# yjb6/SaRO-GS

Measured on AMD Instinct MI355X. Metric: rendered views/s (fwd+bwd) at 1080p vs #Gaussians, higher is better.
Workload: dtype f32; 1 GPU; BASELINE configs[4] stress-1080p: synth(P=3000000, seed 0) SH3, 1920x1080, one view per GPU, fwd+bwd; protocol=SURVEY 8d: 1 / median of per-call device-synchronised wall-clock fwd+bwd, pose_table=off for value (every pose a first visit); on for value_warm, gaussians=3000000, width=1920, height=1080, sh_degree=3, exp_mode=0, poses_per_rank=8, late_gaussians_cold=2255988, word_fork=0

## Files before the change

### saro-gs_amd/csrc/gsrast_binning.h

```cpp
#pragma once
#include "gsrast_common.h"

namespace gsrast {
#define GSRAST_OCC_ATTR(n) __attribute__((amdgpu_waves_per_eu(n, n)))
#ifdef GSRAST_RSCAT_WAVES
#define GSRAST_RSCAT_OCC GSRAST_OCC_ATTR(GSRAST_RSCAT_WAVES)
#else
#define GSRAST_RSCAT_OCC
#endif
#ifdef GSRAST_BSCAT_WAVES
#define GSRAST_BSCAT_OCC GSRAST_OCC_ATTR(GSRAST_BSCAT_WAVES)
#else
#define GSRAST_BSCAT_OCC
#endif
#ifdef GSRAST_BSORT_WAVES
#define GSRAST_BSORT_OCC GSRAST_OCC_ATTR(GSRAST_BSORT_WAVES)
#else
#define GSRAST_BSORT_OCC
#endif
#ifdef GSRAST_EMIT_WAVES
#define GSRAST_EMIT_OCC GSRAST_OCC_ATTR(GSRAST_EMIT_WAVES)
#else
#define GSRAST_EMIT_OCC
#endif
// ... 472 lines not shown
        for (uint32_t c0 = threadIdx.x; c0 < cgx * cgy; c0 += 256 * 4) {
            uint32_t v[4][4];
#pragma unroll
            for (int u = 0; u < 4; u++) {
                const uint32_t c = c0 + u * 256, cx = c % cgx, cy = c / cgx;
#pragma unroll
                for (int k = 0; k < 4; k++) {
                    const uint32_t x = cx * 2u + (k & 1), y = cy * 2u + (k >> 1);
                    v[u][k] = (c < cgx * cgy && x < gx_tiles && y < gy_tiles) ? zcut_used[y * gx_tiles + x] : 0u;
                }
            }
#pragma unroll
            for (int u = 0; u < 4; u++) {
                const uint32_t c = c0 + u * 256;
                const uint32_t m = max(max(v[u][0], v[u][1]), max(v[u][2], v[u][3]));
                if (c < cgx * cgy) s_zc[c] = (uint16_t)(m >= 0xFFFF0000u ? 0xFFFFu : (m + 0xFFFFu) >> 16);
            }
        }
    }
    SCAT_T(1);
    __syncthreads();
    SCAT_T(2);
    const float scale = (float)nb / (float)s_C[ZH_BINS];
    if (blockIdx.x == 0 && threadIdx.x == 0) *zbins_out = s_fl[0] == 0xFFFFu ? 0xFFFFFFFFu : (s_fl[0] | (s_fl[1] << 16));

    uint32_t dg[BK_ITEMS_T], lr[BK_ITEMS_T];
#pragma unroll
    for (int r = 0; r < BK_ITEMS_T; r++) {
        dg[r] = 0u; lr[r] = 0u;
        if (key[r] != 0xFFFFFFFFu) {
            uint32_t bin, pos; int wlog;
            zh_locate(key[r], zh_klo, zh_shift, bin, pos, wlog);
            const float fscale = __uint_as_float((uint32_t)(127 - wlog) << 23);
            const uint32_t fr = pos;
            const uint32_t c0 = s_C[bin], c1 = s_C[bin + 1u];
            const float u = __builtin_fmaf((float)(c1 - c0), fminf((float)fr * fscale, 0.99999994f), (float)c0);
            const uint32_t d = (uint32_t)(u * scale);
            dg[r] = d < nb ? d : nb - 1u;
            const uint32_t cb = COARSE ? dg[r] >> BK_CSHIFT : dg[r];
            const uint32_t sh = (cb & 1u) * 16u;
            lr[r] = (atomicAdd(&cnt[cb >> 1], 1u << sh) >> sh) & 0xFFFFu;
        }
    }
    uint2 rc[BK_ITEMS_T]; uint32_t tl[BK_ITEMS_T];
#pragma unroll
    for (int r = 0; r < BK_ITEMS_T; r++) {
        const uint32_t i = base + r * 256 + threadIdx.x;
        rc[r] = make_uint2(0u, 0u); tl[r] = 0u;
        if (i < n) { rc[r] = rect[i]; tl[r] = tiles[i]; }
    }
    SCAT_T(3);
    __syncthreads();
    SCAT_T(4);
    const uint32_t nres = COARSE ? nb >> BK_CSHIFT : nb;
    uint32_t* gc = gcount + (size_t)xcd * (COARSE ? (uint32_t)BK_NBC_MAX : nb);
    for (uint32_t k0 = threadIdx.x; k0 < nres; k0 += 256 * 16) {
        uint32_t g[16];
#pragma unroll
        for (int u = 0; u < 16; u++) {
            const uint32_t k = k0 + u * 256;
            const uint32_t c = k < nres ? (cnt[k >> 1] >> ((k & 1u) * 16u)) & 0xFFFFu : 0u;
            g[u] = 0xFFFFFFFFu;
            if (c) g[u] = atomicAdd(&gc[k], c);
        }
#pragma unroll
        for (int u = 0; u < 16; u++) {
            const uint32_t mine = g[u] < 0xFFFFu ? g[u] : 0xFFFFu;
            const uint32_t other = (uint32_t)__shfl_xor((int)mine, 1, 64);
            const uint32_t k = k0 + u * 256;
            if (!(threadIdx.x & 1u) && k < nres) cnt[k >> 1] = mine | (other << 16);
        }
    }
    SCAT_T(5);
    __syncthreads();
    SCAT_T(6);
    uint32_t nlate = 0;
#pragma unroll
    for (int r = 0; r < BK_ITEMS_T; r++) {
        bool skipped = true;
        if (key[r] != 0xFFFFFFFFu) {
            uint32_t wword = (rc[r].y & 0xFFFFu) - (rc[r].x & 0xFFFFu);
            if (zcut_used) {
                const uint32_t x0 = rc[r].x & 0xFFFFu, y0 = rc[r].x >> 16, x1 = rc[r].y & 0xFFFFu, y1 = rc[r].y >> 16;
                const uint32_t kq = key[r] >> 16;
                bool late = wword != 0u && (x1 - x0) * (y1 - y0) <= 64u;
                if (late) {
                    const uint32_t cx0 = x0 >> cshift, cx1 = (x1 - 1u) >> cshift, cy0 = y0 >> cshift, cy1 = (y1 - 1u) >> cshift;
                    uint32_t m = 0;
                    if (cx1 - cx0 <= 1u && cy1 - cy0 <= 1u)
                        m = max(max((uint32_t)s_zc[cy0 * cgx + cx0], (uint32_t)s_zc[cy0 * cgx + cx1]), max((uint32_t)s_zc[cy1 * cgx + cx0], (uint32_t)s_zc[cy1 * cgx + cx1]));
                    else
                        for (uint32_t cy = cy0; cy <= cy1; cy++)
                            for (uint32_t cx = cx0; cx <= cx1; cx++) m = max(m, (uint32_t)s_zc[cy * cgx + cx]);
                    late = kq > m;
                }
                if (late) { wword |= LATE_BIT; nlate++; }
            }
            const uint32_t cb = COARSE ? dg[r] >> BK_CSHIFT : dg[r];
            const uint32_t pos = ((cnt[cb >> 1] >> ((cb & 1u) * 16u)) & 0xFFFFu) + lr[r];
            if (COARSE) {
#ifdef GSRAST_SCAT_BATCH_STORES
                rc[r].x = wword | ((dg[r] & ((1u << BK_CSHIFT) - 1u)) << 16);
                lr[r] = pos;
#else
                if (pos < ccap)
                    slab[((size_t)cb * BK_XCD + xcd) * ccap + pos] = make_uint4(key[r], base + r * 256 + threadIdx.x, wword | ((dg[r] & ((1u << BK_CSHIFT) - 1u)) << 16), tl[r]);
#endif
            } else if (pos < (uint32_t)BK_CAPX)
                slab[((size_t)dg[r] * BK_XCD + xcd) * BK_CAPX + pos] = make_uint4(key[r], base + r * 256 + threadIdx.x, wword, tl[r]);
            skipped = (wword & LATE_BIT) != 0u;
        }
        if (color_skip) {
            const unsigned long long m = __ballot(skipped);
            const uint32_t first = base + r * 256 + (threadIdx.x & ~63u);
            if (lane == 0 && first < n) color_skip[first >> 6] = m;
        }
    }
#ifdef GSRAST_SCAT_BATCH_STORES
    if (COARSE) {
#pragma unroll
        for (int r = 0; r < BK_ITEMS_T; r++)
            if (key[r] != 0xFFFFFFFFu && lr[r] < ccap)
                slab[((size_t)(dg[r] >> BK_CSHIFT) * BK_XCD + xcd) * ccap + lr[r]] = make_uint4(key[r], base + r * 256 + threadIdx.x, rc[r].x, tl[r]);
    }
#endif
    if (zcut_used) {
#pragma unroll
        for (int d = 32; d >= 1; d >>= 1) nlate += __shfl_xor(nlate, d, 64);
        if (lane == 0 && nlate) atomicAdd(&s_late, nlate);
        __syncthreads();
        if (threadIdx.x == 0 && s_late) atomicAdd(n_late_out, s_late);
    }
    SCAT_T(7);
#ifdef GSRAST_SCATTER_TIMING
    if (threadIdx.x == 0) atomicMax(&g_scat[13], (unsigned long long)wall_clock64());
#endif
    {
        const uint32_t per = (nb + gridDim.x) / gridDim.x;
        const uint32_t b = blockIdx.x * per + threadIdx.x;
        if (threadIdx.x < per && b <= nb) {
            const float u = (float)b * ((float)s_C[ZH_BINS] / (float)nb);
            uint32_t i = 0;
#pragma unroll
            for (uint32_t st = ZH_BINS / 2; st; st >>= 1) if ((float)s_C[i + st] <= u) i += st;
            const long long k0 = zh_bin_start(i, zh_klo, zh_shift), k1 = zh_bin_start(i + 1u, zh_klo, zh_shift);
            const float c0 = (float)s_C[i], c1 = (float)s_C[i + 1u];
            const float f = fminf(fmaxf((u - c0) / (c1 - c0), 0.0f), 1.0f);
            const long long k = k0 + (long long)(f * (float)(k1 - k0));
            bkey_out[b] = k < 0 ? 0u : (k < (long long)ZH_KEY_TOP ? (uint32_t)k : ZH_KEY_TOP);
        }
    }
}

__global__ void __launch_bounds__(256)
depth_bucket_refine_kernel(const uint4* __restrict__ cslab , const uint32_t* __restrict__ gccount , uint32_t nb,
                           uint32_t* __restrict__ gcount , uint4* __restrict__ slab , uint32_t ccap)
{
    __shared__ uint32_t cnt[1 << BK_CSHIFT];
    const uint32_t x = blockIdx.x & (BK_XCD - 1), c = blockIdx.x >> 3;
    if (threadIdx.x < (1u << BK_CSHIFT)) cnt[threadIdx.x] = 0u;
    const uint32_t n_true = gccount[(size_t)x * BK_NBC_MAX + c];
    const uint32_t n = n_true < ccap ? n_true : ccap;
    const uint4* src = cslab + ((size_t)c * BK_XCD + x) * ccap;
    constexpr int RI = 8;
    __syncthreads();
    for (uint32_t e0 = 0; e0 < n; e0 += RI * 256) {
        uint4 el[RI];
#pragma unroll
        for (int r = 0; r < RI; r++) { const uint32_t e = e0 + r * 256 + threadIdx.x; if (e < n) el[r] = src[e]; }
#pragma unroll
        for (int r = 0; r < RI; r++) {
            const uint32_t e = e0 + r * 256 + threadIdx.x;
            if (e < n) {
                const uint32_t fb = (el[r].z >> 16) & ((1u << BK_CSHIFT) - 1u);
                const uint32_t pos = atomicAdd(&cnt[fb], 1u);
                if (pos < (uint32_t)BK_CAPX)
                    slab[((size_t)((c << BK_CSHIFT) + fb) * BK_XCD + x) * BK_CAPX + pos] = make_uint4(el[r].x, el[r].y, el[r].z & ~BK_FINE_MASK, el[r].w);
            }
        }
    }
    __syncthreads();
    if (threadIdx.x < (1u << BK_CSHIFT))
        gcount[(size_t)x * nb + (c << BK_CSHIFT) + threadIdx.x] = (n_true > ccap && threadIdx.x == 0u) ? 0xFFFFu : cnt[threadIdx.x];
}

__device__ __forceinline__ void wave_sync() { __builtin_amdgcn_fence(__ATOMIC_ACQ_REL, "wavefront"); __builtin_amdgcn_wave_barrier(); }
constexpr int BK_SUB = 256;
constexpr int BK_WAVES = 2;

__device__ __forceinline__ uint4 bucket_element(const uint4* __restrict__ slab, uint32_t b, const uint32_t (&start)[BK_XCD + 1], uint32_t e)
{
    uint32_t x = 0, s0 = 0;
#pragma unroll
    for (int q = 1; q < BK_XCD; q++) { const bool ge = e >= start[q]; x += ge ? 1u : 0u; s0 = ge ? start[q] : s0; }
    return slab[((size_t)b * BK_XCD + x) * BK_CAPX + (e - s0)];
}
__global__ void __launch_bounds__(64 * BK_WAVES) GSRAST_BSORT_OCC
depth_bucket_sort_kernel(const uint4* __restrict__ slab, const uint32_t* __restrict__ gcount, uint32_t nb,
                         const uint32_t* __restrict__ bkey ,
                         uint32_t* __restrict__ border ,
                         uint32_t* __restrict__ bwincl ,
                         uint4* __restrict__ binfo ,
                         uint32_t* __restrict__ bwsum ,
                         uint4* __restrict__ binfo_all = nullptr,
                         const uint32_t* __restrict__ pred = nullptr ,
                         const unsigned long long* __restrict__ keep_bits = nullptr,
                         uint32_t* __restrict__ zero_words = nullptr, uint32_t n_zero_words = 0,
                         uint4* __restrict__ zero_quads = nullptr, uint32_t n_zero_quads = 0)
{
    __shared__ unsigned long long s_grp[BK_WAVES][BK_CAP];
    __shared__ uint16_t s_aux[BK_WAVES][BK_CAP];
    __shared__ uint16_t s_wid[BK_WAVES][BK_CAP];
    __shared__ uint32_t s_cnt[BK_WAVES][BK_SUB + 1];
    if (pred && *pred == 0u) return;
    if (zero_words) for (uint32_t k = blockIdx.x * blockDim.x + threadIdx.x; k < n_zero_words; k += gridDim.x * blockDim.x) zero_words[k] = 0u;
    if (zero_quads) for (uint32_t k = blockIdx.x * blockDim.x + threadIdx.x; k < n_zero_quads; k += gridDim.x * blockDim.x) zero_quads[k] = make_uint4(0u, 0u, 0u, 0u);
    const unsigned lane = lane_id(), wave = threadIdx.x >> 6;
    const uint32_t b = blockIdx.x * BK_WAVES + wave;
    if (b >= nb) return;
    const bool early_only = binfo_all != nullptr;
    unsigned long long* grp = s_grp[wave];
    uint16_t* aux = s_aux[wave];
    uint16_t* wid = s_wid[wave];
    uint32_t* cnt = s_cnt[wave];
    const uint32_t sub_lo = bkey[b], sub_hi = bkey[b + 1u];
    const float sub_scale = (float)BK_SUB / (float)(sub_hi > sub_lo ? sub_hi - sub_lo : 1u);
    auto sub_of = [&](uint32_t key) -> uint32_t {
        if (key <= sub_lo) return 0u;
        const uint32_t d = (uint32_t)((float)(key - sub_lo) * sub_scale);
        return d < (uint32_t)BK_SUB ? d : (uint32_t)BK_SUB - 1u;
    };
    uint32_t c = lane < (unsigned)BK_XCD ? gcount[(size_t)lane * nb + b] : 0u;
    const uint32_t over = __ballot(c > (uint32_t)BK_CAPX) != 0ull ? 1u : 0u;
    c = c < (uint32_t)BK_CAPX ? c : (uint32_t)BK_CAPX;
    uint32_t inc = c;
#pragma unroll
    for (int d = 1; d < BK_XCD; d <<= 1) { const uint32_t t = __shfl_up(inc, d, 64); if (lane >= (unsigned)d) inc += t; }
    uint32_t start[BK_XCD + 1];
    start[0] = 0u;
#pragma unroll
    for (int x = 0; x < BK_XCD; x++) start[x + 1] = __builtin_amdgcn_readlane(inc, x);
    const uint32_t n_all = start[BK_XCD];
    for (uint32_t k = lane; k <= (uint32_t)BK_SUB; k += 64) cnt[k] = 0u;
    wave_sync();
    uint32_t tsum = 0, wall = 0;
    for (uint32_t e0 = lane; e0 < n_all; e0 += 64 * 4) {
        uint4 kv[4];
#pragma unroll
        for (int u = 0; u < 4; u++) { const uint32_t e = e0 + u * 64; kv[u] = e < n_all ? bucket_element(slab, b, start, e) : make_uint4(0u, 0u, 0u, 0u); }
#pragma unroll
        for (int u = 0; u < 4; u++) {
            const uint32_t e = e0 + u * 64;
            if (e < n_all) {
                const bool kept = !(early_only && (kv[u].z & LATE_BIT)) && (!keep_bits || ((keep_bits[kv[u].y >> 6] >> (kv[u].y & 63u)) & 1ull));
                if (!keep_bits || kept) tsum += kv[u].w;
                wall += kv[u].z & ~LATE_BIT;
                if (kept) aux[e] = atomicAdd(&cnt[sub_of(kv[u].x)], 1u);
            }
        }
    }
    wave_sync();
    {
        uint32_t v[BK_SUB / 64], sum = 0;
#pragma unroll
        for (int q = 0; q < BK_SUB / 64; q++) { v[q] = cnt[lane * (BK_SUB / 64) + q]; sum += v[q]; }
        uint32_t run = wave_incl_scan(sum) - sum;
#pragma unroll
        for (int q = 0; q < BK_SUB / 64; q++) { cnt[lane * (BK_SUB / 64) + q] = run; run += v[q]; }
        if (lane == 63) cnt[BK_SUB] = run;
    }
    wave_sync();
    const uint32_t n = cnt[BK_SUB];
    for (uint32_t e0 = lane; e0 < n_all; e0 += 64 * 4) {
        uint4 kv[4];
#pragma unroll
        for (int u = 0; u < 4; u++) { const uint32_t e = e0 + u * 64; kv[u] = e < n_all ? bucket_element(slab, b, start, e) : make_uint4(0u, 0u, 0u, 0u); }
#pragma unroll
        for (int u = 0; u < 4; u++) {
            const uint32_t e = e0 + u * 64;
            if (e < n_all && !(early_only && (kv[u].z & LATE_BIT)) && (!keep_bits || ((keep_bits[kv[u].y >> 6] >> (kv[u].y & 63u)) & 1ull))) {
                const uint32_t slot = cnt[sub_of(kv[u].x)] + aux[e];
                grp[slot] = ((unsigned long long)kv[u].x << 32) | kv[u].y;
                wid[slot] = (uint16_t)(kv[u].z & ~LATE_BIT);
            }
        }
    }
    wave_sync();
    for (uint32_t e = lane; e < n; e += 64) {
        const unsigned long long me = grp[e];
        const uint32_t d2 = sub_of((uint32_t)(me >> 32));
        const uint32_t s0 = cnt[d2], s1 = cnt[d2 + 1];
        uint32_t r = 0;
        for (uint32_t q = s0; q < s1; q++) r += grp[q] < me ? 1u : 0u;
        border[(size_t)b * BK_CAP + s0 + r] = (uint32_t)me;
        aux[s0 + r] = wid[e];
    }
    wave_sync();
    const uint32_t E = (n + 63) / 64;
    uint32_t wsum = 0;
    for (uint32_t e = 0; e < E; e++) { const uint32_t t = lane * E + e; if (t < n) wsum += aux[t]; }
    uint32_t run = wave_incl_scan(wsum) - wsum;
    const uint32_t wtot = __shfl(run + wsum, 63, 64);
#pragma unroll
    for (int d = 32; d >= 1; d >>= 1) { tsum += __shfl_xor(tsum, d, 64); wall += __shfl_xor(wall, d, 64); }
    uint32_t* scanbuf = reinterpret_cast<uint32_t*>(grp);
    for (uint32_t e = 0; e < E; e++) { const uint32_t t = lane * E + e; if (t < n) { run += aux[t]; scanbuf[t] = run; } }
    wave_sync();
    for (uint32_t t = lane; t < n; t += 64) bwincl[(size_t)b * BK_CAP + t] = scanbuf[t];
    if (lane == 0) {
        if (early_only) { binfo[b] = make_uint4(n, wtot, n_all - n, over); binfo_all[b] = make_uint4(n_all, wall, tsum, over); }
        else binfo[b] = make_uint4(n, wtot, tsum, over);
        bwsum[b] = wtot;
    }
}

__device__ __forceinline__ void depth_bucket_totals(const uint4* __restrict__ binfo, uint32_t nb, uint32_t* __restrict__ scalars,
                                                    uint32_t* host_out = nullptr, uint32_t host_seq = 0,
                                                    const uint4* __restrict__ binfo_e = nullptr )
{
    __shared__ unsigned long long s_t[256];
    __shared__ uint32_t s_q[256], s_qe[256];
    uint32_t over = 0, q = 0, qe = 0;
    unsigned long long tsum = 0;
    for (uint32_t k0 = threadIdx.x; k0 < nb; k0 += 256 * 8) {
        uint4 v[8];
#pragma unroll
        for (int u = 0; u < 8; u++) { const uint32_t k = k0 + u * 256; v[u] = k < nb ? binfo[k] : make_uint4(0u, 0u, 0u, 0u); }
#pragma unroll
        for (int u = 0; u < 8; u++) { q += v[u].y; tsum += v[u].z; over |= v[u].w; }
        if (binfo_e) {
#pragma unroll
            for (int u = 0; u < 8; u++) { const uint32_t k = k0 + u * 256; v[u] = k < nb ? binfo_e[k] : make_uint4(0u, 0u, 0u, 0u); }
#pragma unroll
            for (int u = 0; u < 8; u++) qe += v[u].y;
        }
    }
    s_t[threadIdx.x] = tsum; s_q[threadIdx.x] = q; s_qe[threadIdx.x] = qe;
    over = __syncthreads_or((int)over) ? 1u : 0u;
    for (int st = 128; st > 0; st >>= 1) { if ((int)threadIdx.x < st) { s_t[threadIdx.x] += s_t[threadIdx.x + st]; s_q[threadIdx.x] += s_q[threadIdx.x + st]; s_qe[threadIdx.x] += s_qe[threadIdx.x + st]; } __syncthreads(); }
    if (threadIdx.x == 0) {
        scalars[SC_R_LO] = (uint32_t)s_t[0]; scalars[SC_Q] = s_q[0]; scalars[SC_R_HI] = (uint32_t)(s_t[0] >> 32); scalars[SC_BUCKET_OVER] = over;
        const uint32_t q_early = binfo_e ? s_qe[0] : s_q[0], n_late = binfo_e ? scalars[SC_N_LATE] : 0u;
        scalars[SC_Q_EARLY] = q_early;
        scalars[SC_EARLY_COUNTS + SC_R_LO] = (uint32_t)s_t[0]; scalars[SC_EARLY_COUNTS + SC_Q] = q_early; scalars[SC_EARLY_COUNTS + SC_LISTED] = 0u; scalars[SC_EARLY_COUNTS + SC_R_HI] = (uint32_t)(s_t[0] >> 32);
        if (host_out) {
            unsigned long long* h64 = reinterpret_cast<unsigned long long*>(host_out);
            uint32_t vals[SC_BUCKET_OVER + 1];
            vals[SC_R_LO] = (uint32_t)s_t[0]; vals[SC_Q] = s_q[0]; vals[SC_BUCKET_OVER] = over; vals[SC_R_HI] = (uint32_t)(s_t[0] >> 32);
            vals[SC_Q_EARLY] = q_early; vals[SC_N_LATE] = n_late; vals[SC_ZBINS] = scalars[SC_ZBINS];
#pragma unroll
            for (int k = 0; k < RB_WORDS; k++)
                __hip_atomic_store(h64 + k, ((unsigned long long)host_seq << 32) | vals[kReadbackWord[k]], __ATOMIC_RELAXED, __HIP_MEMORY_SCOPE_SYSTEM);
        }
    }
}
__global__ void __launch_bounds__(256)
depth_bucket_scan_kernel(const uint4* __restrict__ binfo, uint32_t nb, uint32_t* __restrict__ scalars )
{
    depth_bucket_totals(binfo, nb, scalars);
}

__global__ void __launch_bounds__(256)
cut_candidates_kernel(uint32_t P, const uint32_t* __restrict__ tiles, const uint2* __restrict__ rect, const unsigned char* __restrict__ need2,
                      uint32_t ntiles, uint32_t gx, unsigned long long* __restrict__ skip, unsigned long long* __restrict__ cand,
                      unsigned long long* __restrict__ skip2, const uint32_t* __restrict__ pred)
{
    __shared__ uint32_t s_need[(BUCKET_MAX_TILES + 32) / 32];
    if (pred && *pred == 0u) return;
    const uint32_t nw = (ntiles + 31u) / 32u;
    for (uint32_t w = threadIdx.x; w < nw; w += 256) {
        uint32_t m = 0;
        for (uint32_t k = 0; k < 32u; k++) { const uint32_t t = w * 32u + k; if (t < ntiles && need2[t]) m |= 1u << k; }
        s_need[w] = m;
    }
    __syncthreads();
    for (uint32_t i0 = blockIdx.x * 256u; i0 < ((P + 63u) & ~63u); i0 += gridDim.x * 256u) {
        const uint32_t i = i0 + threadIdx.x;
        bool c = false;
        if (i < P && tiles[i] != 0u) {
            const uint2 rc = rect[i];
            const uint32_t x0 = rc.x & 0xFFFFu, y0 = rc.x >> 16, x1 = rc.y & 0xFFFFu, y1 = rc.y >> 16;
            if ((x1 - x0) * (y1 - y0) > 1024u) c = true;
            else
                for (uint32_t y = y0; y < y1 && !c; y++)
                    for (uint32_t x = x0; x < x1; x++) { const uint32_t t = y * gx + x; if ((s_need[t >> 5] >> (t & 31u)) & 1u) { c = true; break; } }
        }
        const unsigned long long m = __ballot(c);
        if ((threadIdx.x & 63u) == 0u && i < ((P + 63u) & ~63u)) {
            const unsigned long long old = skip[i >> 6];
            cand[i >> 6] = m;
            skip2[i >> 6] = ~(old & m);
            skip[i >> 6] = old & ~m;
        }
    }
}

template <typename KeyT>
__global__ void __launch_bounds__(256)
emit_instances_kernel(int P, const uint32_t* __restrict__ order, const uint32_t* __restrict__ offsets,
                      const uint32_t* __restrict__ tiles, const uint2* __restrict__ rect, int gx,
                      KeyT* __restrict__ tile_keys, uint32_t* __restrict__ inst_vals)
{
    __shared__ uint32_t s_e[4][64], s_g[4][64], s_xy[4][64], s_w[4][64];
    const int j = blockIdx.x * blockDim.x + threadIdx.x;
    const unsigned lane = lane_id(), wave = threadIdx.x >> 6;
    uint32_t g = 0, cnt = 0, incl, xy = 0, w = 1;
    if (j < P) {
        g = order[j];
        cnt = tiles[g];
        incl = offsets[j];
        if (cnt) {
            const uint2 rc = rect[g];
            xy = rc.x;
            w = (rc.y & 0xFFFFu) - (rc.x & 0xFFFFu);
        }
    } else {
        incl = P > 0 ? offsets[P - 1] : 0u;
    }
    const uint32_t e = incl - cnt;
    const uint32_t wstart = __shfl(e, 0, 64);
    const uint32_t wend = __shfl(incl, 63, 64);
    s_e[wave][lane] = e - wstart; s_g[wave][lane] = g; s_xy[wave][lane] = xy; s_w[wave][lane] = w;
    __syncthreads();
    const uint32_t C = wend - wstart;
    for (uint32_t o = lane; o < C; o += 64) {
        uint32_t sidx = 0;
#pragma unroll
        for (int step = 32; step >= 1; step >>= 1)
            if (s_e[wave][sidx + step] <= o) sidx += step;
        const uint32_t k = o - s_e[wave][sidx];
        const uint32_t ww = s_w[wave][sidx], pxy = s_xy[wave][sidx];
        uint32_t yy = (uint32_t)((float)k * __builtin_amdgcn_rcpf((float)ww));
        if (yy * ww > k) yy--;
        if ((yy + 1) * ww <= k) yy++;
        const uint32_t xx = k - yy * ww;
        tile_keys[wstart + o] = (KeyT)(((pxy >> 16) + yy) * (uint32_t)gx + (pxy & 0xFFFFu) + xx);
        inst_vals[wstart + o] = s_g[wave][sidx];
    }
}

template <typename KeyT>
__global__ void __launch_bounds__(256)
tile_ranges_kernel(uint32_t R, const uint32_t* __restrict__ R_dev ,
                   const KeyT* __restrict__ tile_keys_sorted, uint2* __restrict__ ranges)
{
    const uint32_t i = blockIdx.x * blockDim.x + threadIdx.x;
    if (R_dev) R = *R_dev;
    if (i >= R) return;
    const uint32_t cur = tile_keys_sorted[i];
    if (i == 0) ranges[cur].x = 0;
    else {
        const uint32_t prev = tile_keys_sorted[i - 1];
        if (cur != prev) { ranges[prev].y = i; ranges[cur].x = i; }
    }
    if (i == R - 1) ranges[cur].y = R;
}

__device__ __forceinline__ double sqrt_newton(double x)
{
    const float xf = (float)x;
    if (!(xf > 1e-30f) || !(xf < 1e30f)) return sqrt(x);
    const float s0f = __builtin_sqrtf(xf);
    const double s0 = (double)s0f;
// ... 465 lines not shown
```

### saro-gs_amd/csrc/gsrast_capi.hip

```cpp
#include "gsrast_host.h"
#include "gsrast_common.h"
#include "gsrast_policy.h"
#include "gsrast_preprocess.h"
#include "gsrast_binning.h"
#include "gsrast_blend.h"
#include "gsrast_contrib.h"
#include "gsrast_features.h"
#include "gsrast_distort.h"
#include "gsrast_project.h"
#include "gsrast_exchange.h"

#include <algorithm>
#include <atomic>
#include <chrono>
#include <cstdlib>
#include <thread>
#include <cstdio>
#include <cmath>
#include <cstring>
#include <dlfcn.h>
#ifndef GSRAST_LATE_FILL_WGS
#define GSRAST_LATE_FILL_WGS 256
#endif
#include <mutex>
#include <string>
#include <vector>
#include <unordered_map>

using namespace gsrast;

namespace {

thread_local std::string g_err;
enum OptionKind { OPT_FLAG , OPT_ONE_OF , OPT_CLAMP , OPT_WORD  };
struct OptionRow { const char* name; std::atomic<int>* word; int def; OptionKind kind; int a, b; int gsrast_options::* field ; };
constexpr int OPT_01 = 0b11, OPT_012 = 0b111, OPT_PPL = 0b10111 , OPT_MAX = 0x7FFFFFFF;
constexpr OptionRow kOptions[] = {
    { "exp_mode", &g_opt.exp_mode, 0, OPT_ONE_OF, OPT_012, 0, &gsrast_options::exp_mode },
    { "binning", &g_opt.binning, 0, OPT_ONE_OF, OPT_01, 0, &gsrast_options::binning },
    { "tile_clip", &g_opt.tile_clip, 1, OPT_FLAG, 0, 0, &gsrast_options::tile_clip },
    { "cull", &g_opt.cull, 1, OPT_FLAG, 0, 0, &gsrast_options::cull },
    { "lpt", &g_opt.lpt, 1, OPT_FLAG, 0, 0, &gsrast_options::lpt },
    { "speculative", &g_opt.speculative, 1, OPT_FLAG, 0, 0, &gsrast_options::speculative },
    { "fwd_pixels_per_lane", &g_opt.fwd_pixels_per_lane, 0, OPT_ONE_OF, OPT_PPL, 0, &gsrast_options::fwd_pixels_per_lane },
    { "bwd_pixels_per_lane", &g_opt.bwd_pixels_per_lane, 0, OPT_ONE_OF, OPT_PPL, 0, &gsrast_options::bwd_pixels_per_lane },
    { "sh_grad_factors", &g_opt.sh_grad_factors, 0, OPT_FLAG, 0, 0, &gsrast_options::sh_grad_factors },
    { "side_stream", &g_opt.side_stream, 1, OPT_FLAG, 0, 0, &gsrast_options::side_stream },
    { "depth_sort", &g_opt.depth_sort, 0, OPT_ONE_OF, OPT_01, 0, &gsrast_options::depth_sort },
    { "forward_only", &g_opt.forward_only, 0, OPT_FLAG, 0, 0, &gsrast_options::forward_only },
    { "no_order_hint", &g_opt.no_order_hint, 0, OPT_FLAG, 0, 0, &gsrast_options::no_order_hint },
    { "dense_backward", &g_opt.dense_backward, 0, OPT_FLAG, 0, 0, &gsrast_options::dense_backward },
    { "no_list_cut", &g_opt.no_list_cut, 0, OPT_FLAG, 0, 0, &gsrast_options::no_list_cut },
    { "profile", &g_opt.profile, 0, OPT_WORD, 0, 0, nullptr },
    { "debug_sync", &g_opt.debug_sync, 0, OPT_FLAG, 0, 0, nullptr },
    { "debug_state", &g_opt.debug_state, 0, OPT_FLAG, 0, 0, nullptr },
    { "ablate", &g_opt.ablate, 0, OPT_WORD, 0, 0, nullptr },
    { "mutate", &g_opt.mutate, 0, OPT_WORD, 0, 0, nullptr },
    { "list_cut_always", &g_opt.list_cut_always, 0, OPT_FLAG, 0, 0, nullptr },
    { "chain_gate", &g_opt.chain_gate, 1, OPT_FLAG, 0, 0, nullptr },
    { "touch_bits", &g_opt.touch_bits, 1, OPT_FLAG, 0, 0, nullptr },
    { "sparse_grec", &g_opt.sparse_grec, 1, OPT_FLAG, 0, 0, nullptr },
    { "late_fill_min_p", &g_opt.late_fill_min_p, 750000, OPT_CLAMP, 0, OPT_MAX, nullptr },
    { "tau_sample", &g_opt.tau_sample, 1, OPT_CLAMP, 0, 6, nullptr },
    { "tau_cut", &g_opt.tau_cut, 1, OPT_FLAG, 0, 0, nullptr },
    { "two_level", &g_opt.two_level, 1, OPT_FLAG, 0, 0, nullptr },
    { "two_level_min_p", &g_opt.two_level_min_p, 2500000, OPT_CLAMP, 0, OPT_MAX, nullptr },
    { "sort_hint", &g_opt.sort_hint, 1, OPT_FLAG, 0, 0, nullptr },
    { "bwd_transposed", &g_opt.bwd_transposed, 1, OPT_FLAG, 0, 0, nullptr },
    { "hexplane_scatter", &g_opt.hexplane_scatter, 0, OPT_ONE_OF, OPT_01, 0, nullptr },
};
const OptionRow* option_row(const char* name)
{
    for (const OptionRow& r : kOptions) if (!strcmp(name, r.name)) return &r;
    return nullptr;
}
bool option_take(const OptionRow& r, int value, int* stored)
{
    *stored = r.kind == OPT_FLAG ? (value ? 1 : 0) : r.kind == OPT_CLAMP ? std::min(std::max(value, r.a), r.b) : value;
    return r.kind != OPT_ONE_OF || (value >= 0 && value < 31 && ((r.a >> value) & 1) != 0);
}
PlanSwitches snapshot_switches()
{
    const OptionWords& g = g_opt;
    return PlanSwitches{ g.list_cut_always.load() != 0, g.tau_cut.load() != 0, g.touch_bits.load() != 0, g.sparse_grec.load() != 0, g.two_level.load() != 0, g.chain_gate.load() != 0,
                         g.sort_hint.load() != 0, g.debug_state.load() != 0, g.two_level_min_p.load(), g.tau_sample.load(), g.bwd_transposed.load() != 0, g.late_fill_min_p.load(),
                         g.ablate.load(), g.mutate.load() };
}

const char* const kKernelNames[K_COUNT] = { "preprocess_fwd", "sort_depth", "scan_tiles", "emit_instances",
                                            "sort_tile", "tile_ranges", "blend_fwd", "blend_bwd",
                                            "preprocess_bwd", "mark_visible", "loss_fwd", "loss_bwd", "preprocess_color", "sh_dir_derivs",
                                            "cut_redo" ,
                                            "late_rows_zero" ,
                                            "grec_zero_touched" ,
                                            "densify_classify", "densify_scan", "densify_apply", "densify_stats_update" ,
                                            "contrib_blend", "contrib_finish" ,
                                            "features_fwd", "features_bwd" ,
                                            "distort_fwd", "distort_bwd" ,
                                            "adam_step_visible" ,
                                            "mcmc_plan" , "mcmc_sample" ,
                                            "mcmc_apply" , "mcmc_noise" ,
                                            "mlp_fwd" , "mlp_bwd"  };
thread_local int t_prof_off = 0;
struct Pending { int id; hipEvent_t a, b; };
std::mutex g_prof_mu;
std::vector<Pending> g_pending;
double g_total_ms[K_COUNT];
long long g_launches[K_COUNT];

struct Roctx {
    int (*push)(const char*) = nullptr; int (*pop)() = nullptr;
    Roctx()
    {
        if (!getenv("GSRAST_ROCTX")) return;
        void* h = dlopen("librocprofiler-sdk-roctx.so", RTLD_NOW | RTLD_GLOBAL);
        if (!h) h = dlopen("libroctx64.so", RTLD_NOW | RTLD_GLOBAL);
        if (!h) return;
        push = reinterpret_cast<int (*)(const char*)>(dlsym(h, "roctxRangePushA"));
        pop = reinterpret_cast<int (*)()>(dlsym(h, "roctxRangePop"));
        if (!push || !pop) { push = nullptr; pop = nullptr; }
    }
};
const Roctx& roctx() { static const Roctx r; return r; }
}

namespace gsrast {
OptionWords g_opt;
OptionWords::OptionWords() { for (const OptionRow& r : kOptions) r.word->store(r.def); }
gsrast_options snapshot_defaults()
{
    gsrast_options o{};
    for (const OptionRow& r : kOptions) if (r.field) o.*r.field = r.word->load();
    return o;
}

int fail(int code, const char* what, hipError_t e)
{
    char buf[512];
    if (e != hipSuccess) snprintf(buf, sizeof buf, "%s: %s", what, hipGetErrorString(e));
    else snprintf(buf, sizeof buf, "%s", what);
    g_err = buf;
    return code;
}

RoctxRange::RoctxRange(const char* name) : on(roctx().push != nullptr) { if (on) (void)roctx().push(name); }
RoctxRange::~RoctxRange() { if (on) (void)roctx().pop(); }

ProfScope::ProfScope(int id_, hipStream_t s_) : id(id_), s(s_), on((id_ < 32 ? ((g_opt.profile.load() >> id_) & 1) != 0 : g_opt.profile.load() == -1) && (t_prof_off == 0 || id_ == K_CUT_REDO)), range(kKernelNames[id_])
{
    if (on) { (void)hipEventCreate(&a); (void)hipEventCreate(&b); (void)hipEventRecord(a, s); }
}
ProfScope::~ProfScope()
{
    if (on) {
        (void)hipEventRecord(b, s);
        std::lock_guard<std::mutex> lk(g_prof_mu);
        g_pending.push_back({ id, a, b });
    }
}

int post_launch(const char* what, hipStream_t s)
{
    hipError_t e = hipGetLastError();
    if (e != hipSuccess) return fail(GSRAST_E_DEVICE, what, e);
    static const bool env_sync = getenv("GSRAST_DEBUG_SYNC") != nullptr;
    if (g_opt.debug_sync.load() || env_sync) {
        if (env_sync) fprintf(stderr, "[gsrast] %s\n", what);
        e = hipStreamSynchronize(s);
        if (e != hipSuccess) return fail(GSRAST_E_DEVICE, what, e);
    }
    return GSRAST_OK;
}
}

namespace {
int scan_u32(const uint32_t* src, const uint32_t* idx, uint32_t n, uint32_t* dst, bool inclusive,
             uint32_t* tmp, uint32_t* total_out, hipStream_t s, const uint2* runs = nullptr,
             const uint32_t* aux = nullptr, uint32_t* aux_lo = nullptr, uint32_t* aux_hi = nullptr)
{
    if (n == 0) return GSRAST_OK;
    const uint32_t nb = (n + SC_CHUNK - 1) / SC_CHUNK;
    if (nb == 1 && !aux) {
        scan_apply_kernel<<<1, 256, 0, s>>>(src, idx, runs, n, nullptr, dst, inclusive ? 1 : 0, total_out);
        GS_LAUNCHED("scan_apply");
        return GSRAST_OK;
    }
    scan_block_sums_kernel<<<nb, 256, 0, s>>>(src, idx, runs, n, tmp, aux, tmp + nb);
    GS_LAUNCHED("scan_block_sums");
    scan_single_block_kernel<<<1, 256, 0, s>>>(tmp, nb, aux ? tmp + nb : nullptr, aux_lo, aux_hi);
    GS_LAUNCHED("scan_single_block");
    scan_apply_kernel<<<nb, 256, 0, s>>>(src, idx, runs, n, tmp, dst, inclusive ? 1 : 0, total_out);
    GS_LAUNCHED("scan_apply");
    return GSRAST_OK;
}

template <typename KeyT, typename ValT> struct SortAdapt { KeyT* kC; ValT* vC; uint32_t* block_minmax; uint32_t* sig; bool assume_short; };

template <typename KeyT, typename ValT = uint32_t, int ITEMS = RS_ITEMS>
int radix_sort(KeyT* kA, ValT* vA, KeyT* kB, ValT* vB, uint32_t n, int bits,
               uint32_t* hist, uint32_t* scan_tmp, hipStream_t s,
               const uint2* gather_rect = nullptr, uint32_t* gather_tiles = nullptr, uint32_t* gather_width = nullptr,
               const uint32_t* n_dev = nullptr ,
               const SortAdapt<KeyT, ValT>* ad = nullptr, const uint32_t* pred = nullptr )
{
    if (n == 0) return GSRAST_OK;
    const uint32_t nblk = (n + RS_THREADS * ITEMS - 1) / (RS_THREADS * ITEMS);
    const int passes = radix_passes(bits);
    if (ad && passes == 4 && bits == 32 && nblk > RS_SELF_SCAN_BLOCKS) {
        const uint32_t mask = 255u;
        const int as = ad->assume_short ? RA_ASSUME : 0;
        for (int p = 0; p < (ad->assume_short ? 3 : 4); p++) {
            const int shift = 8 * p;
            const KeyT* kin = (p & 1) ? kB : kA; const ValT* vin = (p & 1) ? vB : vA;
            KeyT* kout = (p & 1) ? kA : kB; ValT* vout = (p & 1) ? vA : vB;
            const int hmode = (p == 0 ? RA_MINMAX : p == 2 ? RA_IN_ALT : p == 3 ? RA_SKIP : 0) | as;
            const int smode = (p == 1 ? RA_OUT_ALT : p == 2 ? (RA_IN_ALT | RA_OUT_ALT | RA_LAST_IF_SHORT) : p == 3 ? RA_SKIP : 0) | as;
            radix_hist_kernel<KeyT, ITEMS><<<nblk, RS_THREADS, 0, s>>>(kin, n, n_dev, shift, mask, hist, nblk, ad->kC, p ? ad->sig : nullptr, hmode, ad->block_minmax);
            GS_LAUNCHED("radix_hist");
            radix_rowscan_kernel<<<mask + 1 + (p == 0 ? 1 : 0), 256, 0, s>>>(hist, nblk, scan_tmp, ad->sig, (p == 0 ? RA_MINMAX : p == 3 ? RA_SKIP : 0) | as, ad->block_minmax, mask + 1);
            GS_LAUNCHED("radix_rowscan");
            radix_scatter_kernel<KeyT, ValT, ITEMS><<<nblk, RS_THREADS, 0, s>>>(kin, vin, kout, vout, n, n_dev, shift, mask, hist, scan_tmp, nblk,
                                                                         p >= 2 ? gather_rect : nullptr, gather_tiles, gather_width,
                                                                         ad->kC, ad->vC, p == 1 ? ad->kC : kA, p == 1 ? ad->vC : vA, ad->sig, smode);
            GS_LAUNCHED("radix_scatter");
        }
        return GSRAST_OK;
    }
    int shift = 0;
    for (int p = 0; p < passes; p++) {
        const int w = (bits - shift + (passes - p) - 1) / (passes - p);
        const uint32_t mask = (1u << w) - 1u;
        radix_hist_kernel<KeyT, ITEMS><<<nblk, RS_THREADS, 0, s>>>(kA, n, n_dev, shift, mask, hist, nblk, nullptr, nullptr, 0, nullptr, pred);
        GS_LAUNCHED("radix_hist");
        const bool self_scan = nblk <= RS_SELF_SCAN_BLOCKS;
        if (!self_scan) {
            radix_rowscan_kernel<<<mask + 1, 256, 0, s>>>(hist, nblk, scan_tmp, nullptr, 0, nullptr, 0, pred);
            GS_LAUNCHED("radix_rowscan");
        }
        const bool last = p == passes - 1;
// ... 376 lines not shown
            blend_fwd_kernel<MODE, PPL><<<grid, 256 / PPL, 0, s>>>(a.ranges, a.plist, a.W, a.H, a.gx, a.T, a.r0, a.r1, a.r2, a.bg, a.oc, a.od, a.fT, a.nc, a.tm, a.bcnt, a.blist);
        });
    });
}

void launch_blend_bwd(int exp_mode, const BlendBwdPick& k, uint32_t grid, hipStream_t s, const BlendArgs& a)
{
    const uint32_t* bcnt = a.from_buckets ? a.bcnt : nullptr;
    auto uncull = [&](auto mode, auto lanes, auto abl) {
        constexpr int PPL = decltype(lanes)::value;
        blend_bwd_kernel<decltype(mode)::value, PPL, decltype(abl)::value><<<grid, 256 / PPL, 0, s>>>(a.ranges, a.plist, a.W, a.H, a.gx, a.T, a.r0, a.r1, a.r2, a.bg, a.fT, a.nc, a.tm, a.dpix, a.grec);
    };
    if (k.ablate) return pick_int<1, 2>(k.ablate, [&](auto abl) { uncull(int_c<0>{}, int_c<4>{}, abl); });
    pick_int<0, 1, 2>(exp_mode, [&](auto mode) {
        constexpr int MODE = decltype(mode)::value;
        if (k.transposed) pick_bool(k.aux, [&](auto aux) { pick_bool(k.abs, [&](auto abs_c) {
            constexpr bool AUX = decltype(aux)::value, ABS = decltype(abs_c)::value;
            blend_bwd_cull_t_kernel<MODE, AUX, ABS><<<grid, 256, 0, s>>>(a.ranges, a.plist, a.order, a.W, a.H, a.gx, a.T, a.r0, a.r1, a.r2, a.bg, a.fT, a.nc, a.tm, a.dpix, a.grec,
                                                                         bcnt, a.blist, AUX ? a.dad : nullptr, AUX ? a.dal : nullptr);
        }); });
        else if (k.cull) pick_int<4, 2, 1>(k.ppl, [&](auto lanes) {
            constexpr int PPL = decltype(lanes)::value;
            blend_bwd_cull_kernel<MODE, PPL><<<grid, 256 / PPL, 0, s>>>(a.ranges, a.plist, a.order, a.W, a.H, a.gx, a.T, a.r0, a.r1, a.r2, a.bg, a.fT, a.nc, a.tm, a.dpix, a.grec, bcnt, a.blist);
        });
        else pick_int<4, 2, 1>(k.ppl, [&](auto lanes) { uncull(mode, lanes, int_c<0>{}); });
    });
}

struct ReplayLaunch {
    int W, H, gx; uint32_t T; unsigned grid;
    const uint2* ranges; const uint32_t* point_list;
    const float4 *rec0, *rec1; const float* final_T; const uint32_t *n_contrib, *tile_max;
    size_t grec;
    ReplayLaunch(int P, int width, int height, const char* geom, const char* binning, const char* image)
    {
        const GeomLayout GL = geom_layout((size_t)P);
        const ImgLayout IL = img_layout((size_t)width, (size_t)height);
        W = width; H = height; gx = (width + TILE_X - 1) / TILE_X;
        T = (uint32_t)gx * (uint32_t)((height + TILE_Y - 1) / TILE_Y); grid = ((T + 7) / 8) * 8;
        ranges = at<uint2>(image, IL.ranges); point_list = at<uint32_t>(binning, 0);
        rec0 = at<float4>(geom, GL.rec0); rec1 = at<float4>(geom, GL.rec1); grec = GL.grec;
        final_T = at<float>(image, IL.final_T); n_contrib = at<uint32_t>(image, IL.n_contrib); tile_max = at<uint32_t>(image, IL.tile_max);
    }
    template <class K, class... A> void front_to_back(K kernel, hipStream_t s, A... own) const
    { kernel<<<grid, 256, 0, s>>>(ranges, point_list, W, H, gx, T, rec0, rec1, n_contrib, tile_max, own...); }
    template <class K, class... A> void back_to_front(K kernel, hipStream_t s, A... own) const
    { kernel<<<grid, 256, 0, s>>>(ranges, point_list, W, H, gx, T, rec0, rec1, final_T, n_contrib, tile_max, own...); }
};

}

extern "C" {

int gsrast_abi_version(void) { return GSRAST_ABI_VERSION; }
const char* gsrast_last_error(void) { return g_err.c_str(); }

void gsrast_options_init(gsrast_options* o)
{
    if (!o) return;
    memset(o, 0, sizeof *o);
    for (const OptionRow& r : kOptions) if (r.field) o->*r.field = r.def;
}
gsrast_context* gsrast_context_create(void) { return new (std::nothrow) gsrast_context(); }
void gsrast_context_destroy(gsrast_context* c)
{
    if (!c) return;
    for (DeviceState& d : c->dev) d.release();
    delete c;
}
int gsrast_context_query(const gsrast_context* c, const char* name)
{
    if (!name) return GSRAST_E_ARG;
    if (!c) c = thread_context();
    if (!strcmp(name, "last_instances")) return (int)c->last_R.load();
    if (!strcmp(name, "last_runs")) return (int)c->last_Q.load();
    if (!strcmp(name, "last_prologue_ns")) return (int)c->last_prologue_ns.load();
    if (!strcmp(name, "redo_count")) return c->redo_count.load();
    if (!strcmp(name, "bucket_skip")) return c->zsort.skip.load();
    if (!strcmp(name, "last_late")) return (int)c->last_late.load();
    if (!strcmp(name, "last_early_runs")) return (int)c->last_Qe.load();
    if (!strcmp(name, "completion_passes")) return (int)c->pol.passes_reported.load();
    if (!strcmp(name, "tau_req")) return c->pol.tau_req.load();
    if (!strcmp(name, "tau_force")) return c->pol.tau_force.load();
    if (!strcmp(name, "cut_margin_x4")) return c->pol.margin.load();
    if (!strcmp(name, "gate_inline_calls")) {
        const int device = current_device();
        return device < 0 ? 0 : (int)c->dev[device].gate.inline_calls;
    }
    if (!strcmp(name, "cut_pause")) return c->pol.pause.load();
    if (!strcmp(name, "cut_fallbacks")) {
        const int device = current_device();
        if (device < 0) return 0;
        if (hipDeviceSynchronize() != hipSuccess) return GSRAST_E_DEVICE;
        uint32_t sum = 0;
        for (const auto& h : c->dev[device].hints) {
            uint32_t v = 0;
            if (h.table && hipMemcpy(&v, &h.table->cut_fallbacks, sizeof v, hipMemcpyDeviceToHost) != hipSuccess) return GSRAST_E_DEVICE;
            sum += v;
        }
        return (int)sum;
    }
    return GSRAST_E_ARG;
}

int gsrast_policy_event(gsrast_context* c, const char* what, int a, int b, int c3)
{
    if (!what) return GSRAST_E_ARG;
    if (!c) c = thread_context();
    CutPolicy& pol = c->pol;
    if (!strcmp(what, "begin")) {
        pol.begin_forward((uint32_t)a);
        c->last_R = (uint32_t)a;
        const bool pays = pol.pays((uint32_t)b, c3 != 0);
        if (!pays) pol.sits_out();
        return pays ? 1 : 0;
    }
    if (!strcmp(what, "counts")) { pol.forward_counts((c3 & 1) != 0, (c3 & 2) ? 1u : 0u, (uint32_t)a, (uint32_t)b, c->last_R.load(), false); return pol.pause.load(); }
    if (!strcmp(what, "pass")) return pol.completion_pass((uint32_t)a, (uint32_t)b, c->last_R.load(), false, c3 != 0);
    if (!strcmp(what, "clean")) { pol.clean_cut_forward(); return pol.fb_score.load(); }
    if (!strcmp(what, "size")) return (int)early_launch_runs((uint32_t)a, (uint32_t)b, c3 != 0);
    if (!strcmp(what, "grow")) return (int)grow_capacity((uint32_t)a);
    if (!strcmp(what, "follow")) return (int)follow_hint((uint32_t)a, (uint32_t)b, c3);
    if (!strcmp(what, "depth_sort")) {
        if (a == 0) c->zsort.radix_forward(); else if (a == 1) c->zsort.clean_forward(); else if (a == 2) (void)c->zsort.overflow(b != 0); else return GSRAST_E_ARG;
        return c->zsort.skip.load();
    }
    if (!strcmp(what, "reset")) { c->pol.~CutPolicy(); new (&c->pol) CutPolicy(); c->zsort.~DepthSortPolicy(); new (&c->zsort) DepthSortPolicy(); return 0; }
    if (!strcmp(what, "tau_min")) { pol.tau_min = std::max(1, a); pol.tau_req = std::max(1, a); return a; }
    if (!strcmp(what, "zrange")) {
        const uint32_t k = c->zrange.klo.load(); const int sh = c->zrange.shift.load();
        const bool held = c->zrange.learn((uint32_t)a, k, sh);
        return c->zrange.shift.load() | (held ? 256 : 0);
    }
    if (!strcmp(what, "zget")) return a == 0 ? (int)(c->zrange.klo.load() >> 8) : a == 1 ? c->zrange.shift.load() : (int)(c->zrange.khi.load() >> 8);
    if (!strcmp(what, "get")) {
        switch (a) { case 0: return pol.pause.load(); case 1: return pol.fb_score.load(); case 2: return pol.margin.load(); case 3: return pol.tau_req.load();
                     case 4: return pol.tau_force.load(); case 5: return pol.fb_pause.load();
                     case 6: return c->zsort.skip.load(); case 7: return c->zsort.backoff.load(); case 8: return c->zsort.clean.load(); default: return GSRAST_E_ARG; }
    }
    return GSRAST_E_ARG;
}

int gsrast_debug_forward_plan(gsrast_context* c, const gsrast_options* options, unsigned flags, int P, int W, int H, const int* words)
{
    if (!options || !words) return fail(GSRAST_E_ARG, "debug_forward_plan: NULL argument");
    if (!c) c = thread_context();
    ForwardPlan p = plan_forward(*options, PlanInputs{ flags, P, W, H, words[4] >> 4, (words[4] & 1) != 0, (words[4] & 2) != 0, words[0], (uint32_t)words[1], (uint32_t)words[2], words[3] != 0 }, snapshot_switches());
    if (p.refusal) return fail(GSRAST_E_ARG, p.refusal);
    p.policy_answer(c->pol.pays(p.last_Q, p.list_cut_always), words[5] != 0);
    const bool bits[] = { p.runbin, p.buckets_ok, p.bucket_sort, p.two_level, p.culled, p.ordered, p.want_hints, p.cut_base, p.tau_mode, p.zero_in_blend, p.zero_touched,
                          p.keep_untouched, p.clip, p.want_shd, p.spec_eligible, p.adaptive_sort, p.assume_short, p.cut_pays, p.cut };
    int v = 0;
    for (size_t k = 0; k < sizeof bits / sizeof bits[0]; k++) v |= bits[k] ? 1 << k : 0;
    return v;
}

int gsrast_debug_backward_plan(const gsrast_options* options, unsigned flags, const int* words, int* grids)
{
    if (!options || !words) return fail(GSRAST_E_ARG, "debug_backward_plan: NULL argument");
    const int in = words[5];
    BackwardInputs bi{ flags, words[0], words[1], words[2], words[3], words[4], (in & 1) != 0, (in & 2) != 0, (in & 4) != 0, (in & 8) != 0, (in & 16) != 0 };
    bi.known_flags = backward_known_flags((in & 32) ? sizeof(gsrast_backward_call) : GSRAST_BACKWARD_CALL_MIN);
    bi.pose_out = (in & 64) != 0; bi.pose_scratch = (in & 128) != 0; bi.abs_sink = (in & 256) != 0;
    BackwardPlan p = plan_backward(*options, bi, snapshot_switches());
    if (p.refusal) return fail(GSRAST_E_ARG, p.refusal);
    p.side_answer(p.wants_side() && words[6] != 0);
    if (grids) { grids[0] = p.derivs_grid; grids[1] = p.per_gaussian_grid; }
    const bool bits[] = { p.aux, p.aa, p.do_blend, p.do_geom, p.zero_records, p.derivs, p.derivs_on_side, p.late_fill_wanted, p.late_fill, p.skip_zero_rows, p.join_late,
                          p.blend, p.pick.cull, p.pick.transposed, p.pick.aux, p.from_buckets, p.tile_order, p.sh_factor, p.factors != 0, p.sparse, p.grouped };
    int v = 0;
    for (size_t k = 0; k < sizeof bits / sizeof bits[0]; k++) v |= bits[k] ? 1 << k : 0;
    return v | p.pick.ppl << 21 | p.pick.ablate << 24 | (p.mutate & 3) << 26 | (p.pose ? 1 << 28 : 0);
}

int gsrast_set_option(const char* name, int value)
{
    if (!name) return GSRAST_E_ARG;
    if (!strcmp(name, "word_fork")) return value == 0 ? 0 : GSRAST_E_ARG;
    const bool both = !strcmp(name, "pixels_per_lane");
    const OptionRow* r = option_row(both ? "fwd_pixels_per_lane" : name);
    int stored = 0;
    if (!r || !option_take(*r, value, &stored)) return GSRAST_E_ARG;
    r->word->store(stored);
    if (both) g_opt.bwd_pixels_per_lane = stored;
    return 0;
}
int gsrast_get_option(const char* name)
{
    if (!name) return GSRAST_E_ARG;
    if (!strcmp(name, "word_fork")) return 0;
    for (const char* word : { "last_instances", "last_runs", "redo_count", "bucket_skip" }) if (!strcmp(name, word)) return gsrast_context_query(nullptr, name);
    const OptionRow* r = option_row(!strcmp(name, "pixels_per_lane") ? "fwd_pixels_per_lane" : name);
    return r ? r->word->load() : GSRAST_E_ARG;
}

int gsrast_profile_kernel_count(void) { return K_COUNT; }
const char* gsrast_profile_kernel_name(int id) { return (id >= 0 && id < K_COUNT) ? kKernelNames[id] : ""; }
int gsrast_profile_collect(void)
{
    std::lock_guard<std::mutex> lk(g_prof_mu);
    for (auto& p : g_pending) {
        float ms = 0.f;
        if (hipEventSynchronize(p.b) == hipSuccess && hipEventElapsedTime(&ms, p.a, p.b) == hipSuccess) {
            g_total_ms[p.id] += ms; g_launches[p.id] += 1;
        }
        (void)hipEventDestroy(p.a); (void)hipEventDestroy(p.b);
    }
    g_pending.clear();
    return 0;
}
int gsrast_profile_read(int id, double* total_ms, long long* launches)
{
    if (id < 0 || id >= K_COUNT) return GSRAST_E_ARG;
    std::lock_guard<std::mutex> lk(g_prof_mu);
    if (total_ms) *total_ms = g_total_ms[id];
    if (launches) *launches = g_launches[id];
    return 0;
}
void gsrast_profile_reset(void)
{
    gsrast_profile_collect();
    std::lock_guard<std::mutex> lk(g_prof_mu);
    for (int i = 0; i < K_COUNT; i++) { g_total_ms[i] = 0; g_launches[i] = 0; }
}

size_t gsrast_geometry_bytes(int P) { return geom_layout((size_t)(P > 0 ? P : 0)).total; }
size_t gsrast_binning_bytes(int R, int, int) { return bin_layout((size_t)(R > 0 ? R : 0)).total; }
size_t gsrast_image_bytes(int W, int H) { return img_layout((size_t)(W > 0 ? W : 0), (size_t)(H > 0 ? H : 0)).total; }
void* gsrast_alloc_prealloc(void* ctx, size_t bytes)
{
    gsrast_prealloc* p = static_cast<gsrast_prealloc*>(ctx);
    if (!p) return nullptr;
    p->requested = bytes;
    return bytes <= p->capacity ? p->ptr : nullptr;
}

int gsrast_mark_visible(int P, const float* means3D, const float* viewmatrix, const float* projmatrix,
                        unsigned char* present, void* stream)
{
    (void)projmatrix;
    hipStream_t s = (hipStream_t)stream;
    if (P < 0 || (P > 0 && (!means3D || !viewmatrix || !present))) return fail(GSRAST_E_ARG, "mark_visible: NULL argument");
    if (P == 0) return GSRAST_OK;
    ProfScope ps(K_MARK_VISIBLE, s);
    mark_visible_kernel<<<(P + 255) / 256, 256, 0, s>>>(P, means3D, viewmatrix, present);
    GS_LAUNCHED("mark_visible");
    return GSRAST_OK;
}

static int prefilter_verdict(const uint32_t* word, hipStream_t s)
{
    uint32_t v = 0;
    GS_HIP(hipMemcpyAsync(&v, word, sizeof v, hipMemcpyDeviceToHost, s));
    GS_HIP(hipStreamSynchronize(s));
    return v ? fail(GSRAST_E_ARG, "forward: a Gaussian passed as prefiltered was culled by the near plane (the reference traps: auxiliary.h:156-160)") : GSRAST_OK;
}

static const char* raw_inputs_check(int P, int M, const gsrast_raw_inputs* in)
{
    if (!in) return "raw: NULL inputs";
    if (P == 0) return nullptr;
    if (!in->xyz || !in->rotation || !in->scaling || !in->opacity_logit || !in->features_dc || (M > 1 && !in->features_rest)) return "raw: NULL required input";
    if (M < 1 || M * 3 > PP_SH_MAX || ((M * 3) & 3)) return "raw: M must be 4 or 16 (SH rows of a multiple of 16 bytes, at most 16 coefficients)";
    if (((uintptr_t)in->rotation | (uintptr_t)in->features_dc | (uintptr_t)in->features_rest | (uintptr_t)in->shs_res) & 15) return "raw: rotation / features_dc / features_rest / shs_res must be 16-byte aligned";
    return nullptr;
}

extern "C++" { namespace {
struct BucketSortArgs {
    const uint4* slab; const uint32_t* gcount; uint32_t nb; const uint32_t* bkey; uint32_t *border, *bwincl; uint4* binfo; uint32_t* bwsum;
    uint4* binfo_all = nullptr;
    const uint32_t* pred = nullptr; const unsigned long long* keep_bits = nullptr;
    uint32_t* zero_words = nullptr; uint32_t n_zero_words = 0; uint4* zero_quads = nullptr; uint32_t n_zero_quads = 0;
};
void launch_bucket_sort(hipStream_t s, const BucketSortArgs& a)
{
    depth_bucket_sort_kernel<<<(a.nb + BK_WAVES - 1) / BK_WAVES, 64 * BK_WAVES, 0, s>>>(a.slab, a.gcount, a.nb, a.bkey, a.border, a.bwincl, a.binfo, a.bwsum, a.binfo_all, a.pred, a.keep_bits,
                                                                                   a.zero_words, a.n_zero_words, a.zero_quads, a.n_zero_quads);
}
struct EmitArgs {
    uint32_t grid; int P; const uint32_t *order, *woffsets; const float4* binrec; int W, H, clip; uint32_t capQ; uint16_t* run_keys; uint2* run_vals;
    const float4 *rec0, *rec1; const uint2* rect;
    const uint4* binfo = nullptr; const uint32_t* bwsum = nullptr; uint32_t nbuckets = 0;
    uint32_t* scalars = nullptr; uint32_t* host_out = nullptr; uint32_t host_seq = 0;
    const uint4* binfo_all = nullptr; const uint32_t* pred = nullptr;
    uint32_t* redo_bucket_cnt = nullptr; int n_redo_cnt = 0; HintTable* redo_hints = nullptr; unsigned long long* host_fallback = nullptr; uint32_t host_fb_seq = 0;
    const unsigned char* need2 = nullptr; int gx_tiles = 0; uint32_t* pass2_counts = nullptr;
};
void launch_emit(hipStream_t s, const EmitArgs& a)
{
    emit_column_runs_kernel<<<a.grid, 256, 0, s>>>(a.P, a.order, a.woffsets, a.binrec, a.W, a.H, a.clip, a.capQ, a.run_keys, a.run_vals, a.binfo, a.bwsum, a.nbuckets, a.scalars,
                                               a.host_out, a.host_seq, a.binfo_all, a.pred, a.redo_bucket_cnt, a.n_redo_cnt, a.redo_hints, a.host_fallback, a.host_fb_seq,
                                               a.need2, a.gx_tiles, a.pass2_counts, a.rec0, a.rec1, a.rect);
}
bool trace_on() { static const bool on = getenv("GSRAST_TRACE") != nullptr; return on; }

struct ForwardRun {
    gsrast_context* const ctx; const gsrast_forward_call& c; const gsrast_options o; const std::chrono::steady_clock::time_point t_entry; const hipStream_t stream;
    const int device; DeviceState* const dev;
    ForwardPlan plan;
    const float *means3D, *shs, *opacities, *scales, *rotations;
    const gsrast_raw_inputs* rawin = nullptr; RawArgs raw{};
    float *out_acc_depth = nullptr, *out_alpha = nullptr;
    int P = 0, W = 0, H = 0; uint32_t T = 0, nbk = 0; CamArgs cam;
    GeomLayout GL; ImgLayout IL; char *geom = nullptr, *img = nullptr, *bin = nullptr; uint32_t cap = 0, capQ = 0;
    float4 *rec0, *rec1, *rec2, *binrec, *grec; uint32_t* tiles; uint2* rect; uint32_t *kA, *kB, *vA, *vB, *offsets, *woffsets, *hist, *scan_tmp, *scalars, *hint_sel, *prefilter_word;
    uint4 *bk_slab, *bk_info, *bk_info_e; uint32_t *bk_count, *bk_key, *bk_order, *bk_wincl, *bk_base, *bk_order_e, *bk_wincl_e, *bk_base_e;
    unsigned long long *color_skip, *cand_bits; unsigned char *untouched = nullptr, *tile_flags; uint32_t* bucket_cnt; uint16_t* bucket_list; uint2* ranges;
    uint32_t *zcut_used = nullptr, *tau_hist = nullptr, *zhist_call = nullptr; TauBins tau_bins{};
    HintTable* hints = nullptr;
    uint32_t zh_klo = 0, zh_wave_mask = 0; int zh_shift = 0;
    uint32_t *zhist_ctx = nullptr, *tau_ctx = nullptr;
    struct SideJoinGuard {
        SideStream* side = nullptr; bool launched = false , joined = false;
        ~SideJoinGuard() { if (launched && side && !joined) (void)hipStreamSynchronize(side->stream); }
    } fork;
    bool bucketed = false;
    bool totals_pending = false;
    bool sort_redone = false;
    Readback *rb_pre = nullptr, *rb_flag = nullptr, *rb = nullptr; uint32_t *pre_alias = nullptr, *flag_alias = nullptr; uint32_t pre_seq = 0, flag_seq = 0;
    ChainGate* gate = nullptr; uint32_t gseq = 0, *gdone = nullptr, *gpred = nullptr;
    uint32_t counts[kCountWords] = { 0 }; uint32_t nQ1 = 0;
    std::chrono::steady_clock::time_point t0, t1;

    ForwardRun(gsrast_context* ctx_, const gsrast_options* options, const gsrast_forward_call& c_, std::chrono::steady_clock::time_point t)
        : ctx(ctx_ ? ctx_ : thread_context()), c(c_), o(options ? *options : snapshot_defaults()), t_entry(t), stream((hipStream_t)c_.stream),
          device(current_device()), dev(ctx->device_state(device)), means3D(c_.means3D), shs(c_.shs), opacities(c_.opacities), scales(c_.scales), rotations(c_.rotations) {}

    int check_and_plan(hipStream_t s)
    {
        P = c.P; W = c.width; H = c.height;
        const bool raw_family = c.family == GSRAST_FAMILY_RAW;
        plan = plan_forward(o, PlanInputs{ c.flags, P, W, H, c.D, (raw_family ? c.raw && c.raw->features_dc : c.shs != nullptr), c.colors_precomp != nullptr,
                                           ctx->zsort.skip.load(), ctx->R_hint.load(), ctx->last_Q.load(), ctx->zsort.depth_short.load() != 0 }, snapshot_switches());
        if (plan.refusal) return fail(GSRAST_E_ARG, plan.refusal);
        if (plan.aux) { out_acc_depth = c.out_acc_depth; out_alpha = c.out_alpha; }
        if (plan.aux && (!out_acc_depth || !out_alpha)) return fail(GSRAST_E_ARG, "forward: NULL acc_depth / alpha output");
        if (raw_family) {
            rawin = c.raw;
            if (const char* e = raw_inputs_check(P, c.M, rawin)) return fail(GSRAST_E_ARG, e);
            means3D = rawin->xyz; shs = rawin->features_dc ; opacities = rawin->opacity_logit; scales = rawin->scaling; rotations = rawin->rotation;
            raw.motion_res = rawin->motion_res; raw.rot_res = rawin->rot_res; raw.trbf = rawin->trbf; raw.opacity_logit = rawin->opacity_logit;
            raw.features_dc = rawin->features_dc; raw.features_rest = rawin->features_rest; raw.shs_res = rawin->shs_res;
        }
        if (P < 0 || W <= 0 || H <= 0 || c.D < 0 || c.D > 3) return fail(GSRAST_E_ARG, "forward: bad P / image size / SH degree");
        if (!c.geometry_alloc || !c.binning_alloc || !c.image_alloc) return fail(GSRAST_E_ARG, "forward: NULL allocator");
        if (!c.out_color || !c.out_depth || !c.background) return fail(GSRAST_E_ARG, "forward: NULL output / background");
        const size_t N = (size_t)W * H;
        if (P == 0) {
            GS_HIP(hipMemsetAsync(c.out_color, 0, 3 * N * sizeof(float), s));
            GS_HIP(hipMemsetAsync(c.out_depth, 0, N * sizeof(float), s));
            if (plan.aux) { GS_HIP(hipMemsetAsync(out_acc_depth, 0, N * sizeof(float), s)); GS_HIP(hipMemsetAsync(out_alpha, 0, N * sizeof(float), s)); }
            return 0;
        }
        if (!means3D || !opacities || !c.viewmatrix || !c.projmatrix || !c.radii) return fail(GSRAST_E_ARG, "forward: NULL required input");
        if (!shs && !c.colors_precomp) return fail(GSRAST_E_ARG, "forward: need shs or colors_precomp");
        if (!c.cov3D_precomp && (!scales || !rotations)) return fail(GSRAST_E_ARG, "forward: need scales+rotations or cov3D_precomp");
        if (shs && !c.colors_precomp && (!c.cam_pos || c.M < (c.D + 1) * (c.D + 1))) return fail(GSRAST_E_ARG, "forward: SH path needs campos and M >= (D+1)^2");
        return GSRAST_OK;
    }

    int buffers(hipStream_t s)
    {
        cam = make_cam(c.viewmatrix, c.projmatrix, c.cam_pos, c.tan_fovx, c.tan_fovy, c.scale_modifier, W, H);
        T = plan.T;
        GL = geom_layout((size_t)P);
        geom = (char*)c.geometry_alloc(c.geometry_ctx, GL.total);
        if (!geom) return fail(GSRAST_E_ALLOC, "forward: geometry allocation failed");
        IL = img_layout((size_t)W, (size_t)H);
        img = (char*)c.image_alloc(c.image_ctx, IL.total);
        if (!img) return fail(GSRAST_E_ALLOC, "forward: image allocation failed");
        rec0 = at<float4>(geom, GL.rec0); rec1 = at<float4>(geom, GL.rec1); rec2 = at<float4>(geom, GL.rec2); grec = at<float4>(geom, GL.grec);
        tiles = at<uint32_t>(geom, GL.tiles); rect = at<uint2>(geom, GL.rect);
        kA = at<uint32_t>(geom, GL.keyA); kB = at<uint32_t>(geom, GL.keyB); vA = at<uint32_t>(geom, GL.valA); vB = at<uint32_t>(geom, GL.valB);
        offsets = at<uint32_t>(geom, GL.offsets); woffsets = at<uint32_t>(geom, GL.woffsets); hist = at<uint32_t>(geom, GL.hist); scan_tmp = at<uint32_t>(geom, GL.scan_tmp);
        scalars = at<uint32_t>(geom, GL.scalars); hint_sel = scalars + HINT_SEL;
        bk_slab = at<uint4>(geom, GL.bk_slab); bk_info = at<uint4>(geom, GL.bk_info); bk_info_e = at<uint4>(geom, GL.bk_info_e);
        bk_count = at<uint32_t>(geom, GL.bk_count); bk_key = at<uint32_t>(geom, GL.bk_key);
        bk_order = at<uint32_t>(geom, GL.bk_order); bk_wincl = at<uint32_t>(geom, GL.bk_wincl); bk_base = at<uint32_t>(geom, GL.bk_base);
        bk_order_e = at<uint32_t>(geom, GL.bk_order_e); bk_wincl_e = at<uint32_t>(geom, GL.bk_wincl_e); bk_base_e = at<uint32_t>(geom, GL.bk_base_e);
        color_skip = at<unsigned long long>(geom, GL.color_skip); cand_bits = at<unsigned long long>(geom, GL.cand_bits);
        tile_flags = at<unsigned char>(img, IL.tile_flags); bucket_cnt = at<uint32_t>(img, IL.bucket_cnt); bucket_list = at<uint16_t>(img, IL.bucket_list);
        ranges = at<uint2>(img, IL.ranges);
        prefilter_word = c.prefiltered ? scalars + SC_PREFILTER : nullptr;
        if (prefilter_word) GS_HIP(hipMemsetAsync(prefilter_word, 0, sizeof(uint32_t), s));
        nbk = depth_buckets_host((size_t)P);
        zh_klo = ctx->zrange.klo.load(); zh_shift = ctx->zrange.shift.load();
        while ((((size_t)P + 63) / 64) / ((size_t)zh_wave_mask + 1) > 1024) zh_wave_mask = 2u * zh_wave_mask + 1u;
        if (o.side_stream && dev) fork.side = dev->side_stream(ctx->mu);
        return GSRAST_OK;
    }

    int begin_policy(hipStream_t s)
    {
        hints = plan.want_hints && dev ? dev->hint_table(ctx->mu, T, s) : nullptr;
        CutPolicy& pol = ctx->pol;
        if (pol.begin_forward((uint32_t)P)) {
            std::lock_guard<std::mutex> lk(ctx->mu);
            if (hints)
                for (auto& h : dev->hints) if (h.table) GS_HIP(hipMemsetAsync(h.table, 0, sizeof(HintTable) , s));
            ctx->pose_seen.clear(); ctx->Qe_hint = 0; ctx->Qe_hint_tau = 0;
        }
        plan.policy_answer(pol.pays(plan.last_Q, plan.list_cut_always), hints != nullptr);
        binrec = plan.cut ? nullptr : at<float4>(geom, GL.binrec);
        if (!plan.cut && !o.no_list_cut) pol.sits_out();
        const bool forced = plan.cut && plan.tau_mode && pol.forced_prediction();
        bool pose_expected = false;
        if (plan.cut && plan.tau_mode && hints && !forced) { std::lock_guard<std::mutex> lk(ctx->mu); auto it = ctx->pose_seen.find(c.viewmatrix); pose_expected = it != ctx->pose_seen.end() && it->second != 0; }
        plan.prediction_answer(forced, pose_expected);
        tau_hist = plan.tau_on ? at<uint32_t>(img, IL.tau_hist) : nullptr;
        tau_bins = TauBins{0u, 0.0f, 0.0f, plan.tau_sample_mask};
        {   const uint32_t klo = ctx->zrange.klo.load(), khi = ctx->zrange.khi.load();
            if (plan.tau_on && khi > klo + (uint32_t)TAU_BINS) { tau_bins.lo = klo; tau_bins.scale = (float)TAU_BINS / (float)(khi - klo); tau_bins.inv_scale = (float)(khi - klo) / (float)TAU_BINS; } }
        zcut_used = plan.cut ? at<uint32_t>(img, IL.zcut_used) : nullptr;
        untouched = plan.keep_untouched ? at<unsigned char>(geom, GL.untouched) : nullptr;
        if (plan.cut) rb_pre = read_flag_prepare(device, &pre_alias, &pre_seq);
        return GSRAST_OK;
    }

    int preprocess(hipStream_t s)
    {
        ProfScope ps(K_PREPROCESS_FWD, s);
        const int pf_grid = (P + PF_THREADS - 1) / PF_THREADS;
        float* cov_dbg = plan.debug_state ? at<float>(geom, GL.cov3D) : nullptr;
        if (plan.bucket_sort) {
            zhist_call = zhist_ctx = dev ? dev->depth_hist(ctx->mu) : nullptr;
            if (!zhist_call) {
                zhist_call = at<uint32_t>(geom, GL.zhist);
                GS_HIP(hipMemsetAsync(zhist_call, 0, ZH_COPIES * ZH_BINS * sizeof(uint32_t), s));
            }
        }
        if (tau_hist) {
            const size_t words = (size_t)TAU_COPIES * T * TAU_BINS;
            if (plan.bucket_sort && zhist_ctx && !plan.debug_state  && (words & 3) == 0 && words / 4 <= 0xFFFFFFFFull)
                tau_ctx = dev->mass_table(ctx->mu, words, s);
            if (tau_ctx) tau_hist = tau_ctx; else GS_HIP(hipMemsetAsync(tau_hist, 0, words * sizeof(uint32_t), s));
        }
        const int nzero = plan.bucket_sort ? (int)nbk * BK_XCD + BK_XCD * BK_NBC_MAX : 0;
        unsigned long long* host_found = rb_pre ? reinterpret_cast<unsigned long long*>(pre_alias) + RB_FOUND : nullptr;
        pick_bool(rawin != nullptr, [&](auto raw_c) { pick_bool(plan.aa, [&](auto aa_c) {
            preprocess_fwd_kernel<decltype(raw_c)::value, decltype(aa_c)::value><<<pf_grid, PF_THREADS, 0, s>>>(
                P, means3D, scales, rotations, opacities, raw, c.cov3D_precomp, cam, c.radii, rec0, rec1, cov_dbg,
                tiles, rect, binrec, kA, plan.bucket_sort ? nullptr : vA, plan.clip ? 1 : 0, bucket_cnt, zhist_call, zh_klo, zh_shift, zh_wave_mask, bk_count, nzero, hints, hint_sel,
                zcut_used, T, scalars, host_found, pre_seq, prefilter_word, untouched, tau_hist, tau_bins);
        }); });
        GS_LAUNCHED("preprocess_fwd");
        ctx->last_prologue_ns = (uint32_t)std::min<long long>(std::chrono::duration_cast<std::chrono::nanoseconds>(std::chrono::steady_clock::now() - t_entry).count(), 0xFFFFFFFFll);
        if (tau_hist) {
            const dim3 tg((unsigned)((cam.gx + TAU_TILE - 1) / TAU_TILE), (unsigned)((cam.gy + TAU_TILE - 1) / TAU_TILE));
            tau_cut_kernel<<<tg, TAU_BLK * TAU_BLK, 0, s>>>(tau_hist, T, cam.gx, cam.gy, tau_bins, (uint32_t)ctx->pol.tau_req.load() * 256u, hints ? hint_sel : nullptr, plan.tau_forced ? 1 : 0,
                                              zcut_used, tau_bins.scale > 0.0f ? 0 : 1);
            GS_LAUNCHED("tau_cut");
        }
        return GSRAST_OK;
    }

    BucketSortArgs whole_buckets() const { return BucketSortArgs{ bk_slab, bk_count, nbk, bk_key, bk_order, bk_wincl, bk_info, bk_base }; }
    int sort_and_scan(hipStream_t s, bool assume, bool buckets)
    {
        bucketed = buckets; totals_pending = false;
        if (buckets) {
            ProfScope ps(K_SORT_DEPTH, s);
            const int items = depth_scatter_items((size_t)P);
            const bool two = plan.two_level;
            auto scatter = two ? (items == BK_ITEMS_WIDE ? depth_bucket_scatter_kernel<BK_ITEMS_WIDE, true> : depth_bucket_scatter_kernel<BK_ITEMS, true>)
                               : (items == BK_ITEMS_WIDE ? depth_bucket_scatter_kernel<BK_ITEMS_WIDE, false> : depth_bucket_scatter_kernel<BK_ITEMS, false>);
            uint4* cslab = reinterpret_cast<uint4*>(grec);
            const uint32_t ccap = depth_coarse_cap((size_t)P, nbk);
            uint32_t* gccount = at<uint32_t>(geom, GL.bk_ccount);
            scatter<<<(P + 256 * items - 1) / (256 * items), 256, 0, s>>>(kA, rect, tiles, (uint32_t)P, zhist_call, zh_klo, zh_shift, nbk, two ? gccount : bk_count, two ? cslab : bk_slab, bk_key, scalars + SC_ZBINS,
                                                                           zcut_used, T, (uint32_t)cam.gx, scalars + SC_N_LATE, plan.cut ? color_skip : nullptr, (uint32_t)plan.cut_cs, ccap);
            GS_LAUNCHED("depth_bucket_scatter");
            if (two) {
                depth_bucket_refine_kernel<<<(nbk >> BK_CSHIFT) * BK_XCD, 256, 0, s>>>(cslab, gccount, nbk, bk_count, bk_slab, ccap);
                GS_LAUNCHED("depth_bucket_refine");
            }
            BucketSortArgs a = whole_buckets();
            if (plan.cut) { a.border = bk_order_e; a.bwincl = bk_wincl_e; a.binfo = bk_info_e; a.bwsum = bk_base_e; a.binfo_all = bk_info; }
            a.zero_words = zhist_ctx; a.n_zero_words = ZH_COPIES * ZH_BINS;
            if (tau_ctx) { a.zero_quads = reinterpret_cast<uint4*>(tau_ctx); a.n_zero_quads = (uint32_t)((size_t)TAU_COPIES * T * TAU_BINS / 4); }
            launch_bucket_sort(s, a);
            GS_LAUNCHED("depth_bucket_sort");
            if (a.zero_quads) { std::lock_guard<std::mutex> lk(ctx->mu); dev->tau_dirty = false; }
            totals_pending = true;
            return GSRAST_OK;
        }
        {   ProfScope ps(K_SORT_DEPTH, s);
            if (plan.bucket_sort) {
                iota_kernel<<<(P + 255) / 256, 256, 0, s>>>(vA, (uint32_t)P);
                GS_LAUNCHED("iota");
            }
            const SortAdapt<uint32_t, uint32_t> ad{ at<uint32_t>(geom, GL.keyC), at<uint32_t>(geom, GL.valC), at<uint32_t>(geom, GL.sort_minmax), scalars + SC_SIG, assume };
            int rc = radix_sort<uint32_t, uint32_t, GSRAST_DEPTH_ITEMS>(kA, vA, kB, vB, (uint32_t)P, 32, hist, scan_tmp, s, rect, plan.runbin ? nullptr : offsets, woffsets, nullptr, &ad);
            if (rc != GSRAST_OK) return rc;
        }
        ProfScope ps(K_SCAN_TILES, s);
        if (plan.runbin)
            return scan_u32(woffsets, nullptr, (uint32_t)P, woffsets, true, scan_tmp, scalars + SC_Q, s, nullptr, tiles, scalars + SC_R_LO, scalars + SC_R_HI);
        int rc = scan_u32(offsets, nullptr, (uint32_t)P, offsets, true, scan_tmp, scalars + SC_R_LO, s);
        if (rc != GSRAST_OK) return rc;
        return scan_u32(woffsets, nullptr, (uint32_t)P, woffsets, true, scan_tmp, scalars + SC_Q, s);
    }

    void learn_pose()
    {
        plan.pose_answer(!(plan.cut && rb_pre && hints) || read_found(rb_pre));
        if (plan.cut && plan.tau_mode && hints && rb_pre) {
            std::lock_guard<std::mutex> lk(ctx->mu);
            if (ctx->pose_seen.size() > 4096) ctx->pose_seen.clear();
            ctx->pose_seen[c.viewmatrix] = plan.pose_known ? 1 : 0;
        }
    }
    size_t bin_bytes() const { return plan.runbin ? runbin_layout((size_t)cap, (size_t)capQ).total : bin_layout((size_t)cap).total; }
    int speculative_buffer(hipStream_t s)
    {
        if (!plan.runbin) GS_HIP(hipMemsetAsync(ranges, 0, (size_t)T * sizeof(uint2), s));
        t0 = std::chrono::steady_clock::now();
        if (plan.R_hint) {
            cap = grow_capacity(plan.R_hint); capQ = grow_capacity(ctx->Q_hint.load());
            bin = (char*)c.binning_alloc(c.binning_ctx, bin_bytes());
            if (!bin) cap = capQ = 0;
        }
        t1 = std::chrono::steady_clock::now();
        plan.binning_answer(bin != nullptr);
        return GSRAST_OK;
    }

    int color_kernels(hipStream_t cs, bool early_only, const uint32_t* pred)
    {
        ProfScope ps(K_COLOR, cs);
        const float* const colors_precomp = c.colors_precomp; const float* const cam_pos = c.cam_pos; const int D = c.D, M = c.M;
        float4 *sA = plan.want_shd ? at<float4>(geom, GL.shdA) : nullptr, *sB = plan.want_shd ? at<float4>(geom, GL.shdB) : nullptr; float* sC = plan.want_shd ? at<float>(geom, GL.shdC) : nullptr;
        const float* sh_in = colors_precomp ? nullptr : shs;
        unsigned char* cl = at<unsigned char>(geom, GL.clamped);
        float4* gz = (fork.side || plan.zero_in_blend) ? nullptr : grec;
        const bool staged = sh_in && M * 3 <= PP_SH_MAX && ((M * 3) & 3) == 0 && ((uintptr_t)sh_in & 15) == 0;
        const int grid = (P + PP_THREADS - 1) / PP_THREADS;
        if (early_only) {
            const unsigned char* skip = at<unsigned char>(geom, pred ? GL.skip2 : GL.color_skip);
            const int cgrid = (P + PCC_IDS - 1) / PCC_IDS;
            if (rawin) preprocess_color_compact_kernel<true><<<cgrid, 64 * PCC_WAVES, 0, cs>>>(P, D, M, means3D, nullptr, nullptr, raw, cam_pos, rec2, cl, sA, sB, sC, skip, pred);
            else preprocess_color_compact_kernel<false><<<cgrid, 64 * PCC_WAVES, 0, cs>>>(P, D, M, means3D, sh_in, colors_precomp, raw, cam_pos, rec2, cl, sA, sB, sC, skip, pred);
        } else if (rawin) {
            if (M * 3 == PP_SH_MAX) preprocess_color_kernel<PP_SH_MAX, true><<<grid, PP_THREADS, 0, cs>>>(P, D, M, means3D, nullptr, raw, cam_pos, rec2, cl, gz, sA, sB, sC, pred);
            else preprocess_color_kernel<0, true><<<grid, PP_THREADS, 0, cs>>>(P, D, M, means3D, nullptr, raw, cam_pos, rec2, cl, gz, sA, sB, sC, pred);
        } else if (staged && M * 3 == PP_SH_MAX)
            preprocess_color_kernel<PP_SH_MAX, false><<<grid, PP_THREADS, 0, cs>>>(P, D, M, means3D, sh_in, raw, cam_pos, rec2, cl, gz, sA, sB, sC, pred);
        else if (staged)
            preprocess_color_kernel<0, false><<<grid, PP_THREADS, 0, cs>>>(P, D, M, means3D, sh_in, raw, cam_pos, rec2, cl, gz, sA, sB, sC, pred);
        else
            preprocess_color_direct_kernel<<<(P + 255) / 256, 256, 0, cs>>>(P, D, M, means3D, sh_in, colors_precomp, cam_pos, rec2, cl, gz, sA, sB, sC, pred);
        hipError_t e = hipGetLastError();
        if (e != hipSuccess) return fail(GSRAST_E_DEVICE, "preprocess_color", e);
        return GSRAST_OK;
    }
    int launch_color(hipStream_t s)
    {
        if (fork.launched) return GSRAST_OK;
        fork.launched = true;
        SideStream* const side = fork.side;
        if (side) {
            GS_HIP(hipEventRecord(side->fork, s));
            GS_HIP(hipStreamWaitEvent(side->stream, side->fork, 0));
        }
        { int rc = color_kernels(side ? side->stream : s, plan.cut_colors, nullptr); if (rc != GSRAST_OK) return rc; }
        if (side) {
            GS_HIP(hipEventRecord(side->join, side->stream));
            if (!plan.zero_in_blend) {
                GS_HIP(hipMemsetAsync(grec, 0, (size_t)P * GREC * sizeof(float), side->stream));
                GS_HIP(hipEventRecord(side->join2, side->stream));
            }
        }
        return GSRAST_OK;
    }

    int run_binning(hipStream_t s, uint32_t nQ, const uint32_t* counts_dev, int mode, const uint32_t* pred, bool readback_after_emit)
    {
        const RunBinLayout RL = runbin_layout((size_t)cap, (size_t)capQ);
        uint16_t *rkA = at<uint16_t>(bin, RL.rkeyA), *rkB = at<uint16_t>(bin, RL.rkeyB);
        uint2 *rvA = at<uint2>(bin, RL.rvalA), *rvB = at<uint2>(bin, RL.rvalB);
        uint32_t *hist_x = at<uint32_t>(bin, RL.hist_x), *hist_y = at<uint32_t>(bin, RL.hist_y), *rscan = at<uint32_t>(bin, RL.scan_tmp), *plist_w = at<uint32_t>(bin, RL.point_list);
        const uint32_t* Q_dev = counts_dev ? counts_dev + SC_Q : nullptr;
        const int xbits = tile_bits((size_t)cam.gx);
        {   ProfScope ps(K_EMIT, s);
            EmitArgs e{};
            e.grid = nbk + 1; e.P = P; e.order = bk_order; e.woffsets = bk_wincl; e.binrec = binrec; e.W = W; e.H = H; e.clip = o.tile_clip; e.capQ = capQ; e.run_keys = rkA; e.run_vals = rvA;
            e.rec0 = rec0; e.rec1 = rec1; e.rect = rect;
            if (bucketed) { e.binfo = bk_info; e.bwsum = bk_base; e.nbuckets = nbk; }
            if (bucketed && mode == 1) {
                e.order = bk_order_e; e.woffsets = bk_wincl_e; e.binfo = bk_info_e; e.bwsum = bk_base_e; e.binfo_all = bk_info;
                e.scalars = scalars; e.host_out = flag_alias; e.host_seq = flag_seq;
            } else if (bucketed && mode == 2) {
                BucketSortArgs a = whole_buckets(); a.pred = pred; a.keep_bits = cand_bits;
                launch_bucket_sort(s, a);
                e.pred = pred; e.redo_bucket_cnt = bucket_cnt; e.n_redo_cnt = XCD_GROUPS * WORK_BUCKETS ; e.redo_hints = hints;
                e.host_fallback = rb_pre ? reinterpret_cast<unsigned long long*>(pre_alias) + RB_FALLBACK : nullptr; e.host_fb_seq = pre_seq;
                e.need2 = tile_flags; e.gx_tiles = cam.gx; e.pass2_counts = scalars + SC_PASS2;
            } else if (bucketed) {
                if (plan.cut) {
                    launch_bucket_sort(s, whole_buckets());
                    GS_LAUNCHED("depth_bucket_sort");
                }
                e.scalars = scalars; e.host_out = flag_alias; e.host_seq = flag_seq;
            } else { e.grid = (uint32_t)((P + 255) / 256); e.order = vA; e.woffsets = woffsets; }
            launch_emit(s, e);
            GS_LAUNCHED("emit_column_runs"); }
        if (bucketed && mode != 2) totals_pending = false;
        if (readback_after_emit) { int rc = read_u32_begin(device, scalars, s, kCountWords, &rb); if (rc != GSRAST_OK) return rc; }
        const uint32_t nblk = (nQ + RUNS_PER_BLOCK - 1) / RUNS_PER_BLOCK;
        ProfScope ps(K_SORT_TILE, s);
        int rc = radix_sort<uint16_t, uint2, GSRAST_RUN_SORT_ITEMS>(rkA, rvA, rkB, rvB, nQ, xbits, hist_x, rscan, s, nullptr, nullptr, nullptr, Q_dev, nullptr, pred);
        if (rc != GSRAST_OK) return rc;
        if (radix_passes(xbits) & 1) { std::swap(rkA, rkB); std::swap(rvA, rvB); }
        run_hist_rows_kernel<<<nblk, 256, 0, s>>>(rvA, nQ, Q_dev, hist_y, nblk, (uint32_t)cam.gy, pred);
        GS_LAUNCHED("run_hist_rows");
        radix_rowscan_kernel<<<cam.gy, 256, 0, s>>>(hist_y, nblk, rscan, nullptr, 0, nullptr, 0, pred);
        GS_LAUNCHED("radix_rowscan");
        rows_and_ranges_kernel<<<nblk + (uint32_t)cam.gx, RS_THREADS, 0, s>>>(rkA, rvA, nQ, counts_dev, cap, tile_bits((size_t)cam.gy), cam.gx, cam.gy, hist_y, rscan, nblk,
                                                                             mode == 2 ? plist_w + cap : plist_w, scalars + (mode == 2 ? SC_PASS2 : 0) + SC_LISTED, ranges,
                                                                             plan.buckets_ok ? bucket_cnt : nullptr, bucket_list, hints, hint_sel, pred,
                                                                             mode == 2 ? tile_flags : nullptr, mode == 2 ? cap : 0u,
                                                                             (mode == 1 && plan.tau_on) ? zcut_used : nullptr);
        GS_LAUNCHED("rows_and_ranges");
        return GSRAST_OK;
    }
    template <typename KeyT> int instance_binning(hipStream_t s, uint32_t R)
    {
        const BinLayout BL = bin_layout((size_t)cap);
        uint32_t *tkA = at<uint32_t>(bin, BL.keyA), *tkB = at<uint32_t>(bin, BL.keyB);
        uint32_t *tvA = at<uint32_t>(bin, BL.valA), *tvB = at<uint32_t>(bin, BL.valB);
        if (tile_passes(T) & 1) { std::swap(tkA, tkB); std::swap(tvA, tvB); }
        KeyT *hA = reinterpret_cast<KeyT*>(tkA), *hB = reinterpret_cast<KeyT*>(tkB);
        { ProfScope ps(K_EMIT, s);
          emit_instances_kernel<KeyT><<<(P + 255) / 256, 256, 0, s>>>(P, vA, offsets, tiles, rect, cam.gx, hA, tvA);
          GS_LAUNCHED("emit_instances"); }
        { ProfScope ps(K_SORT_TILE, s);
          int rc = radix_sort<KeyT>(hA, tvA, hB, tvB, R, tile_bits(T), at<uint32_t>(bin, BL.hist), at<uint32_t>(bin, BL.scan_tmp), s);
          if (rc != GSRAST_OK) return rc; }
        ProfScope ps(K_RANGES, s);
        tile_ranges_kernel<KeyT><<<(R + 255) / 256, 256, 0, s>>>(R, nullptr, reinterpret_cast<const KeyT*>(at<uint32_t>(bin, BL.keyA)), ranges);
        GS_LAUNCHED("tile_ranges");
        return GSRAST_OK;
    }

    void claim_gate()
    {
        if (!plan.chain_gate || counter_collection_env() || !dev || (gate = dev->chain_gate(ctx->mu, device)) == nullptr) return;
        std::lock_guard<std::mutex> lk(ctx->mu);
        uint32_t n = gate->seq + 1u; if (n == 0u) n = 1u;
        bool free_slot = true;
        for (uint32_t back = GATE_RING / 2u; back <= GATE_RING; back++) {
            const uint32_t k = n - back;
            if (k != 0u && gate->tail_seq[k % GATE_RING] == k) { free_slot = hipEventQuery(gate->tail[k % GATE_RING]) == hipSuccess; break; }
        }
        if (!free_slot) { gate->inline_calls++; gate = nullptr; return; }
        gate->seq = n; gseq = n; gate->tail_seq[n % GATE_RING] = 0u;
        gdone = gate->words + (gseq % GATE_RING); gpred = gate->words + GATE_RING + (gseq % GATE_RING);
    }
    int blend(hipStream_t s, const uint32_t* plist, bool fwd_lists_built, int mode, const uint32_t* pred)
    {
        { int rc = launch_color(s); if (rc != GSRAST_OK) return rc; }
        SideStream* const side = fork.side;
        if (side) { GS_HIP(hipStreamWaitEvent(s, side->join, 0)); if (plan.zero_in_blend) fork.joined = true; }
        ProfScope ps(K_BLEND_FWD, s);
        uint32_t grid = ((T + 7) / 8) * 8;
        BlendArgs ba{};
        ba.ranges = ranges; ba.plist = plist; ba.W = W; ba.H = H; ba.gx = cam.gx; ba.T = T; ba.r0 = rec0; ba.r1 = rec1; ba.r2 = rec2;
        ba.bg = c.background; ba.oc = c.out_color; ba.od = c.out_depth; ba.fT = at<float>(img, IL.final_T); ba.nc = at<uint32_t>(img, IL.n_contrib); ba.tm = at<uint32_t>(img, IL.tile_max);
        ba.oad = out_acc_depth; ba.oal = out_alpha;
        if (plan.zero_in_blend && !plan.zero_touched && !o.forward_only && mode != 2) { ba.zero4 = grec; ba.n_zero4 = (uint32_t)((size_t)P * 4); }
        if (fwd_lists_built) { ba.hints = hints; ba.hint_sel = hint_sel; }
        ba.cut_margin_x4 = (uint32_t)ctx->pol.margin.load();
        ba.untouched = untouched;
        if (mode == 1) { ba.zcut_used = zcut_used; ba.cut_scalars = scalars; ba.tile_flags = tile_flags; }
        if (mode == 1 && plan.culled) claim_gate();
        if (mode == 1 && gate) ba.gate = GateArgs{ bucket_cnt + (XCD_GROUPS + 1) * WORK_BUCKETS, gpred, gdone, gseq };
        if (mode == 2) ba.pred = pred;
        if (plan.buckets_ok) { ba.bcnt = bucket_cnt; ba.blist = bucket_list; }
        if (plan.ordered) {
            if (plan.buckets_ok && fwd_lists_built) { ba.from_buckets = 1; grid = (uint32_t)(XCD_GROUPS * xcd_group_tiles_host((size_t)cam.gx, (size_t)cam.gy)); }
            else {
                uint32_t* ord = at<uint32_t>(img, IL.order_fwd);
                tile_order_kernel<<<1, 1024, 0, s>>>(T, ranges, nullptr, ord);
                GS_LAUNCHED("tile_order");
                ba.order = ord;
            }
        }
        launch_blend_fwd(o.exp_mode, plan.culled, o.fwd_pixels_per_lane ? o.fwd_pixels_per_lane : 1 , grid, s, ba);
        GS_LAUNCHED("blend_fwd");
        if (side && !plan.zero_in_blend) { GS_HIP(hipStreamWaitEvent(s, side->join2, 0)); fork.joined = true; }
        return GSRAST_OK;
    }

    int speculative_launch(hipStream_t s)
    {
        if (!(plan.speculative && totals_pending)) {
            if (totals_pending) {
                ProfScope ps(K_SCAN_TILES, s);
                depth_bucket_scan_kernel<<<1, 256, 0, s>>>(bk_info, nbk, scalars);
                GS_LAUNCHED("depth_bucket_scan");
                totals_pending = false;
            }
            int rc = read_u32_begin(device, scalars, s, kCountWords, &rb); if (rc != GSRAST_OK) return rc;
        }
        if (!plan.speculative) return GSRAST_OK;
        const bool late = totals_pending;
        if (late) { if (rb_pre) { rb_flag = rb_pre; flag_alias = pre_alias; flag_seq = pre_seq; } else rb_flag = read_flag_prepare(device, &flag_alias, &flag_seq); }
        if (plan.cut) nQ1 = early_launch_runs(early_hint().load(), capQ, plan.pose_known || plan.tau_on);
        int rc = run_binning(s, plan.cut ? nQ1 : capQ, plan.cut ? scalars + SC_EARLY_COUNTS : scalars, plan.cut ? 1 : 0, nullptr, late && !rb_flag);
        flag_alias = nullptr;
        if (rc == GSRAST_OK) rc = blend(s, at<uint32_t>(bin, 0), true, plan.cut ? 1 : 0, nullptr);
        return rc;
    }
    std::atomic<uint32_t>& early_hint() const { return (plan.tau_on && (plan.tau_forced || !plan.pose_known || !hints)) ? ctx->Qe_hint_tau : ctx->Qe_hint; }

    int sort_again(hipStream_t s)
    {
        ctx->redo_count++;
        int rc = sort_and_scan(s, false, false);
        if (rc == GSRAST_OK) rc = read_u32(device, scalars, s, counts, kCountWords);
        sort_redone = true;
        return rc;
    }
    int absorb_depth_sort(hipStream_t s)
    {
        { int rc = rb_flag ? read_flag_finish(rb_flag, scalars, s, counts) : read_u32_finish(rb, scalars, s, counts, kCountWords); if (rc != GSRAST_OK) return rc; }
        DepthSortPolicy& zs = ctx->zsort;
        if (!plan.bucket_sort && o.depth_sort == 0) zs.radix_forward();
        if (plan.bucket_sort) {
            if (counts[SC_BUCKET_OVER] == 0) zs.clean_forward();
            else {
                zs.overflow(ctx->zrange.learn(counts[SC_ZBINS], zh_klo, zh_shift));
                int rc = sort_again(s); if (rc != GSRAST_OK) return rc;
                if (plan.adaptive_sort) zs.radix_key_bits(counts[SC_KEY_BITS]);
            }
        } else if (plan.adaptive_sort) {
            if (plan.assume_short && counts[SC_SHORT_WRONG] != 0) { int rc = sort_again(s); if (rc != GSRAST_OK) return rc; }
            zs.radix_key_bits(counts[SC_KEY_BITS]);
        }
        if (plan.runbin && counts[SC_R_HI] != 0) return fail(GSRAST_E_OVERFLOW, "forward: more than 2^31-1 instances");
        return GSRAST_OK;
    }
    int absorb_counts()
    {
        const auto t2 = std::chrono::steady_clock::now();
        CutPolicy& pol = ctx->pol;
        if (trace_on()) fprintf(stderr, "[gsrast] alloc(spec) %.1f us, readback wait %.1f us, cap %u R %u Q %u%s | cut %d (pays %d: last_Q %u pause %d) late %u Q_early %u nQ1 %u capQ %u bucket_sort %d (over %u) hints %d zh %08x >> %d bins %u-%u\n",
                               std::chrono::duration<double, std::micro>(t1 - t0).count(), std::chrono::duration<double, std::micro>(t2 - t1).count(), cap, counts[SC_R_LO], counts[SC_Q],
                               plan.speculative ? " (speculative)" : "", (int)plan.cut, (int)plan.cut_pays, ctx->last_Q.load(), pol.pause.load(), counts[SC_N_LATE], counts[SC_Q_EARLY], nQ1, capQ,
                               (int)plan.bucket_sort, counts[SC_BUCKET_OVER], hints ? 1 : 0, zh_klo, zh_shift, counts[SC_ZBINS] & 0xFFFFu, counts[SC_ZBINS] >> 16);
        if (counts[SC_R_LO] > 0x7FFFFFFFu) return fail(GSRAST_E_OVERFLOW, "forward: more than 2^31-1 instances");
        const uint32_t R = counts[SC_R_LO], Q = counts[SC_Q];
        if (plan.bucket_sort && !sort_redone) (void)ctx->zrange.learn(counts[SC_ZBINS], zh_klo, zh_shift);
        ctx->R_hint = follow_hint(ctx->R_hint.load(), R, 4); ctx->Q_hint = follow_hint(ctx->Q_hint.load(), Q, 4);
        ctx->last_R = R; ctx->last_Q = Q;
        ctx->last_late = plan.cut ? counts[SC_N_LATE] : 0u; ctx->last_Qe = plan.cut ? counts[SC_Q_EARLY] : Q;
        if (plan.cut) pol.forward_counts(plan.tau_on, counts[SC_N_LATE], Q, counts[SC_Q_EARLY], (uint32_t)P, plan.list_cut_always);
        if (plan.cut && plan.speculative && !sort_redone) { std::atomic<uint32_t>& hint = early_hint(); hint = follow_hint(hint.load(), counts[SC_Q_EARLY], 5); }
        if (const uint32_t q2 = take_fallback_event(device)) {
            const int before = pol.fb_score.load();
            const int pts = pol.completion_pass(q2, ctx->last_Q.load(), (uint32_t)P, plan.list_cut_always, plan.tau_mode);
            if (trace_on()) fprintf(stderr, "[gsrast] completion pass reported: %u column runs of %u, %d points on a score of %d; margin %d / 4, tau_req %d, pause %d\n", q2, ctx->last_Q.load(), pts, before,
                                   pol.margin.load(), pol.tau_req.load(), pol.pause.load());
        } else if (plan.cut && counts[SC_N_LATE] != 0u) pol.clean_cut_forward();
        return GSRAST_OK;
    }

    int completion_pass(hipStream_t s_caller)
    {
        if (gate) {
            GS_HIP(hipEventRecord(gate->ev, s_caller));
            GS_HIP(hipStreamWaitEvent(gate->stream, gate->ev, 0));
        }
        const hipStream_t s = gate ? gate->stream : s_caller;
        const uint32_t* const pred = gate ? gpred : scalars + SC_REDO_PRED;
        ProfScope ps(K_CUT_REDO, s);
        struct Off { Off() { t_prof_off++; } ~Off() { t_prof_off--; } } off;
        cut_candidates_kernel<<<std::min((P + 255) / 256, 2048), 256, 0, s>>>((uint32_t)P, tiles, rect, tile_flags, T, (uint32_t)cam.gx, color_skip, cand_bits, at<unsigned long long>(geom, GL.skip2), pred);
        int rc = post_launch("cut_candidates", s);
        if (rc == GSRAST_OK && plan.cut_colors) rc = color_kernels(s, true, pred);
        if (rc == GSRAST_OK) rc = run_binning(s, capQ, scalars + SC_PASS2, 2, pred, false);
        if (rc == GSRAST_OK) rc = blend(s, at<uint32_t>(bin, 0), true, 2, pred);
        if (gate) {
            chain_done_kernel<<<1, 1, 0, gate->stream>>>(pred, gdone, gseq);
            const hipError_t e1 = hipGetLastError();
            {   std::lock_guard<std::mutex> lk(ctx->mu);
                if (hipEventRecord(gate->tail[gseq % GATE_RING], gate->stream) == hipSuccess) gate->tail_seq[gseq % GATE_RING] = gseq; }
            const hipError_t e2 = hipStreamWaitValue32(s_caller, gdone, gseq, hipStreamWaitValueEq, 0xFFFFFFFFu);
            if (e1 != hipSuccess || e2 != hipSuccess) {
                { std::lock_guard<std::mutex> lk(ctx->mu); gate->failed = true; }
                (void)hipEventRecord(gate->ev, gate->stream);
                (void)hipStreamWaitEvent(s_caller, gate->ev, 0);
            }
        }
        return rc;
    }
    int finish(hipStream_t s, uint32_t R)
    {
        if (plan.zero_touched) {
            ProfScope ps(K_GREC_ZERO, s);
            grec_zero_touched_kernel<<<(unsigned)(((size_t)P + 256 * GZ_PER - 1) / (256 * GZ_PER)), 256, 0, s>>>(P, untouched, grec, scalars);
            GS_LAUNCHED("grec_zero_touched");
        }
        if (prefilter_word) { int rc = prefilter_verdict(prefilter_word, s); if (rc != GSRAST_OK) return rc; }
        return (int)R;
    }
    int exact_redo(hipStream_t s, uint32_t R, uint32_t Q)
    {
        if (plan.speculative && !sort_redone) ctx->redo_count++;
        if (plan.cut) GS_HIP(hipMemsetAsync(scalars + SC_N_LATE, 0, sizeof(uint32_t), s));
        if (plan.cut_colors && fork.launched) {
            if (fork.side) GS_HIP(hipStreamWaitEvent(s, fork.side->join, 0));
            int rc = color_kernels(s, false, nullptr);
            if (rc != GSRAST_OK) return rc;
        }
        if (plan.speculative)
            GS_HIP(hipMemsetAsync(bucket_cnt, 0, (XCD_GROUPS + 1) * WORK_BUCKETS * sizeof(uint32_t), s));
        if (!bin || R > cap || Q > capQ) {
            cap = R; capQ = Q;
            bin = (char*)c.binning_alloc(c.binning_ctx, bin_bytes());
            if (!bin) return fail(GSRAST_E_ALLOC, "forward: binning allocation failed");
        }
        if (plan.runbin && (R == 0 || Q == 0)) GS_HIP(hipMemsetAsync(ranges, 0, (size_t)T * sizeof(uint2), s));
        int rc = GSRAST_OK;
        if (R > 0 && Q > 0 && plan.runbin) rc = run_binning(s, Q, nullptr, 0, nullptr, false);
        else if (R > 0 && !plan.runbin) rc = T <= 65536u ? instance_binning<uint16_t>(s, R) : instance_binning<uint32_t>(s, R);
        if (rc == GSRAST_OK) rc = blend(s, at<uint32_t>(bin, 0), plan.runbin && R > 0 && Q > 0, 0, nullptr);
        return rc == GSRAST_OK ? finish(s, R) : rc;
    }
};
} }

static int forward_impl(gsrast_context* ctx, const gsrast_options* options, const gsrast_forward_call& c)
{
    const auto t_entry = std::chrono::steady_clock::now();
    RoctxRange range_fwd(c.family == GSRAST_FAMILY_RAW ? "gsrast_forward" "_raw" : "gsrast_forward");
    ForwardRun r(ctx, options, c, t_entry);
    const hipStream_t s = r.stream;
    int rc = r.check_and_plan(s);
    if (rc != GSRAST_OK || c.P == 0) return rc;
    if ((rc = r.buffers(s)) != GSRAST_OK || (rc = r.begin_policy(s)) != GSRAST_OK) return rc;
    if ((rc = r.preprocess(s)) != GSRAST_OK || (rc = r.sort_and_scan(s, r.plan.assume_short, r.plan.bucket_sort)) != GSRAST_OK) return rc;
    r.learn_pose();
    if ((rc = r.speculative_buffer(s)) != GSRAST_OK || (rc = r.launch_color(s)) != GSRAST_OK || (rc = r.speculative_launch(s)) != GSRAST_OK) return rc;
    if ((rc = r.absorb_depth_sort(s)) != GSRAST_OK || (rc = r.absorb_counts()) != GSRAST_OK) return rc;
    const ForwardPlan& plan = r.plan;
    const uint32_t R = r.counts[SC_R_LO], Q = r.counts[SC_Q];
    const bool early_fits = !plan.cut || r.counts[SC_Q_EARLY] <= r.nQ1;
    if (!(plan.speculative && !r.sort_redone && R <= r.cap && Q <= r.capQ && early_fits)) return r.exact_redo(s, R, Q);
    if (plan.cut && r.counts[SC_N_LATE] != 0u && (rc = r.completion_pass(s)) != GSRAST_OK) return rc;
    return r.finish(s, R);
}

static const char* take_record(void* own, size_t own_size, const void* call, size_t min_size)
{
    if (!call) return "call record: NULL";
    size_t n;
    memcpy(&n, call, sizeof n);
    if (n < min_size || n > own_size) return "call record: struct_size is not one this library knows";
    memset(own, 0, own_size);
    memcpy(own, call, n);
    return nullptr;
}
static bool family_known(int family) { return family == GSRAST_FAMILY_DENSE || family == GSRAST_FAMILY_RAW; }

int gsrast_render_forward(gsrast_context* ctx, const gsrast_options* options, const gsrast_forward_call* call)
{
    gsrast_forward_call c;
    if (const char* e = take_record(&c, sizeof c, call, GSRAST_FORWARD_CALL_MIN)) return fail(GSRAST_E_ARG, e);
    if (!family_known(c.family)) return fail(GSRAST_E_ARG, "call record: unknown family");
    if (c.family == GSRAST_FAMILY_DENSE ? c.raw != nullptr
                                        : c.means3D || c.shs || c.colors_precomp || c.opacities || c.scales || c.rotations || c.cov3D_precomp || c.prefiltered)
        return fail(GSRAST_E_ARG, "call record: dense family with raw set, or raw family with a dense input / prefiltered set");
    return forward_impl(ctx, options, c);
}

int gsrast_forward(gsrast_alloc_fn geometry_alloc, void* geometry_ctx, gsrast_alloc_fn binning_alloc,
                   void* binning_ctx, gsrast_alloc_fn image_alloc, void* image_ctx, int P, int D, int M,
                   const float* background, int width, int height, const float* means3D, const float* shs,
                   const float* colors_precomp, const float* opacities, const float* scales,
                   float scale_modifier, const float* rotations, const float* cov3D_precomp,
                   const float* viewmatrix, const float* projmatrix, const float* cam_pos, float tan_fovx,
                   float tan_fovy, int prefiltered, float* out_color, float* out_depth, int* radii, void* stream)
{
    gsrast_forward_call c{};
    c.struct_size = sizeof c; c.family = GSRAST_FAMILY_DENSE;
    c.geometry_alloc = geometry_alloc; c.geometry_ctx = geometry_ctx; c.binning_alloc = binning_alloc; c.binning_ctx = binning_ctx;
    c.image_alloc = image_alloc; c.image_ctx = image_ctx;
    c.P = P; c.D = D; c.M = M; c.background = background; c.width = width; c.height = height;
    c.means3D = means3D; c.shs = shs; c.colors_precomp = colors_precomp; c.opacities = opacities; c.scales = scales;
    c.rotations = rotations; c.cov3D_precomp = cov3D_precomp; c.scale_modifier = scale_modifier;
    c.viewmatrix = viewmatrix; c.projmatrix = projmatrix; c.cam_pos = cam_pos; c.tan_fovx = tan_fovx; c.tan_fovy = tan_fovy;
    c.prefiltered = prefiltered; c.out_color = out_color; c.out_depth = out_depth; c.radii = radii; c.stream = stream;
    return forward_impl(nullptr, nullptr, c);
}

__global__ void __launch_bounds__(256)
touched_rows_kernel(int P, const unsigned char* __restrict__ untouched, const uint32_t* __restrict__ scalars, unsigned char* __restrict__ flags)
{
    const int i = blockIdx.x * 256 + threadIdx.x;
    if (i >= P) return;
    flags[i] = scalars[SC_TOUCH_VALID] != 0u ? (unsigned char)(untouched[i] ? 0 : 1) : (unsigned char)1;
}
int gsrast_touched_rows(int P, const char* geom_buffer, unsigned char* flags, void* stream)
{
    hipStream_t s = (hipStream_t)stream;
    if (P < 0 || (P > 0 && (!geom_buffer || !flags))) return fail(GSRAST_E_ARG, "touched_rows: bad arguments");
    if (P == 0) return GSRAST_OK;
    const GeomLayout GL = geom_layout((size_t)P);
    touched_rows_kernel<<<(P + 255) / 256, 256, 0, s>>>(P, at<unsigned char>(geom_buffer, GL.untouched), at<uint32_t>(geom_buffer, GL.scalars), flags);
    GS_LAUNCHED("touched_rows");
    return GSRAST_OK;
}

namespace {
struct ContribLayout { size_t sum, max, cnt, top, total; };
ContribLayout contrib_layout(size_t P)
{
    ContribLayout L; Carver c;
    const size_t Pp = P ? P : 1;
    L.sum = c.take(Pp * 8); L.max = c.take(Pp * 4); L.cnt = c.take(Pp * 4); L.top = c.take(Pp * 4);
    L.total = c.o;
    return L;
}
}

size_t gsrast_contrib_scratch_bytes(int P) { return contrib_layout(P > 0 ? (size_t)P : 0).total; }

int gsrast_contrib_stats(const gsrast_options* options, int P, int R, int width, int height, const char* geom_buffer, const char* binning_buffer,
                         const char* image_buffer, const float* pixel_weights, float* stats, char* scratch, void* stream)
{
    hipStream_t s = (hipStream_t)stream;
// ... 591 lines not shown
```

### saro-gs_amd/csrc/gsrast_common.h

```cpp
#pragma once
#include <hip/hip_runtime.h>
#include "gsrast_host.h"
#include <stdint.h>
#include <stddef.h>

namespace gsrast {

constexpr int TILE_X = 16;
constexpr int TILE_Y = 16;
constexpr int TILE_PIX = TILE_X * TILE_Y;
constexpr int WAVE = 64;

#ifndef GSRAST_REC_STRIDE
#define GSRAST_REC_STRIDE 1
#endif
constexpr int REC_STRIDE = GSRAST_REC_STRIDE;
struct GeomLayout {
    size_t rec0, rec1, rec2, cov3D, clamped, tiles, rect, binrec, keyA, keyB, valA, valB, offsets, woffsets,
        hist, scan_tmp, scalars, grec, keyC, valC, sort_minmax, shdA, shdB, shdC, zhist, bk_key, bk_count, bk_ccount , bk_slab, bk_order, bk_wincl, bk_info, bk_base,
        bk_order_e, bk_wincl_e, bk_info_e, bk_base_e ,
        color_skip ,
        cand_bits ,
        skip2 ,
        untouched , total;
};
constexpr int GREC = 16;
constexpr size_t BUCKET_SORT_MIN_P = 32768;
#ifndef GSRAST_BK_TARGET
#define GSRAST_BK_TARGET 256
#endif
#ifndef GSRAST_BK_CAP
#define GSRAST_BK_CAP 1024
#endif
constexpr int ZH_BINS = 1024, ZH_COPIES = 8 ;
constexpr int ZH_TAIL = 64, ZH_MID = ZH_BINS - 2 * ZH_TAIL, ZH_TAIL_LOG = 4;
constexpr uint32_t ZH_KLO_DEFAULT = 0x3E400000u;
constexpr int ZH_SHIFT_DEFAULT = 21;
constexpr uint32_t ZH_KEY_TOP = 0x7F800000u;
__host__ __device__ inline void zh_locate(uint32_t key, uint32_t kmid, int shift, uint32_t& bin, uint32_t& pos, int& wlog)
{
    const int d = (int)key - (int)kmid;
    const int wt = shift + ZH_TAIL_LOG;
    if (d < 0) {
        wlog = wt;
        const uint32_t m = (uint32_t)(-d - 1), t = m >> wt, w1 = (1u << wt) - 1u;
        if (t >= (uint32_t)ZH_TAIL) { bin = 0u; pos = 0u; }
        else { bin = (uint32_t)(ZH_TAIL - 1) - t; pos = w1 - (m & w1); }
    } else if (((uint32_t)d >> shift) < (uint32_t)ZH_MID) {
        wlog = shift;
        bin = (uint32_t)ZH_TAIL + ((uint32_t)d >> shift); pos = (uint32_t)d & ((1u << shift) - 1u);
    } else {
        wlog = wt;
        const uint32_t e = (uint32_t)d - ((uint32_t)ZH_MID << shift), t = e >> wt, w1 = (1u << wt) - 1u;
        if (t >= (uint32_t)ZH_TAIL) { bin = (uint32_t)ZH_BINS - 1u; pos = w1; }
        else { bin = (uint32_t)(ZH_TAIL + ZH_MID) + t; pos = e & w1; }
    }
}
__host__ __device__ inline long long zh_bin_start(uint32_t bin, uint32_t kmid, int shift)
{
    if (bin < (uint32_t)ZH_TAIL) return (long long)kmid - ((long long)((uint32_t)ZH_TAIL - bin) << (shift + ZH_TAIL_LOG));
    if (bin < (uint32_t)(ZH_TAIL + ZH_MID)) return (long long)kmid + ((long long)(bin - (uint32_t)ZH_TAIL) << shift);
    return (long long)kmid + ((long long)ZH_MID << shift) + ((long long)(bin - (uint32_t)(ZH_TAIL + ZH_MID)) << (shift + ZH_TAIL_LOG));
}
static inline uint32_t depth_buckets_host(size_t P)
{
    uint32_t nb = 256;
    while ((size_t)nb * GSRAST_BK_TARGET < P && nb < 8192u) nb <<= 1;
    return nb;
}
struct BinLayout {
    size_t keyA, keyB, valA, valB, hist, scan_tmp, total;
};
struct ImgLayout {
    size_t final_T, n_contrib, ranges, tile_max, order_fwd, order_bwd, bucket_cnt, bucket_list, zcut_used ,
        tile_flags ,
        tau_hist , total;
};
constexpr int WORK_BUCKETS = 64;
constexpr size_t BUCKET_MAX_TILES = 65535;
constexpr int XCD_GROUPS = 8;
static inline size_t xcd_group_tiles_host(size_t gx, size_t gy) { return gx * ((gy + XCD_GROUPS - 1) / XCD_GROUPS); }

constexpr int HINT_SLOTS = 256;
struct HintTable {
    uint32_t key[HINT_SLOTS][2];
    uint32_t stamp[HINT_SLOTS];
    uint32_t clock, cut_fallbacks , pad[2];
};
constexpr int SC_R_LO = 0;
constexpr int SC_Q = 1;
constexpr int SC_LISTED = 2;
constexpr int SC_R_HI = 3;
constexpr int SC_Q_EARLY = 4;
constexpr int SC_N_LATE = 5;
constexpr int SC_UNDONE = 6, SC_REDO_PRED = SC_UNDONE;
constexpr int SC_ZBINS = 7;
constexpr int SC_SIG = 8;
constexpr int SIG_BITS = 0, SIG_BASE = 1, SIG_WRONG = 2;
constexpr int SC_KEY_BITS = SC_SIG + SIG_BITS;
constexpr int SC_KEY_BASE = SC_SIG + SIG_BASE;
constexpr int SC_SHORT_WRONG = SC_SIG + SIG_WRONG;
constexpr int SC_BUCKET_OVER = 11;
constexpr int HINT_SEL = 16;
constexpr int SC_EARLY_COUNTS = 20;
constexpr int SC_PASS2 = 24;
constexpr int SC_GATE_COUNT = 28;
constexpr int HINT_PUB = 32;
constexpr int SC_PREFILTER = 44;
constexpr int SC_TOUCH_VALID = 45;
constexpr int SC_GREC_SPARSE = 46;
constexpr int kReadbackWord[] = { SC_R_LO, SC_Q, SC_BUCKET_OVER, SC_R_HI, SC_Q_EARLY, SC_N_LATE, SC_ZBINS };
constexpr int RB_WORDS = (int)(sizeof kReadbackWord / sizeof kReadbackWord[0]);
constexpr int RB_FOUND = 7;
constexpr int RB_FALLBACK = 8;
__host__ __device__ inline uint16_t* hint_work(HintTable* h, uint32_t) { return reinterpret_cast<uint16_t*>(h + 1); }
__host__ __device__ inline const uint16_t* hint_work(const HintTable* h, uint32_t) { return reinterpret_cast<const uint16_t*>(h + 1); }
static inline size_t hint_zcut_offset(size_t T) { return (sizeof(HintTable) + (size_t)HINT_SLOTS * T * 2 + 255) & ~(size_t)255; }
__host__ __device__ inline uint32_t* hint_zcut(HintTable* h, uint32_t T) { return reinterpret_cast<uint32_t*>(reinterpret_cast<char*>(h) + ((sizeof(HintTable) + (size_t)HINT_SLOTS * T * 2 + 255) & ~(size_t)255)); }
__host__ __device__ inline const uint32_t* hint_zcut(const HintTable* h, uint32_t T) { return reinterpret_cast<const uint32_t*>(reinterpret_cast<const char*>(h) + ((sizeof(HintTable) + (size_t)HINT_SLOTS * T * 2 + 255) & ~(size_t)255)); }
static inline size_t hint_table_bytes(size_t T) { return hint_zcut_offset(T) + (size_t)HINT_SLOTS * T * 4 + 256; }

constexpr uint32_t ZCUT_NONE = 0xFFFFFFFFu;
constexpr uint32_t CUT_MAX_CELLS = 3072;
static inline int cut_cell_shift(size_t gx, size_t gy)
{
    if (gx >= 32768) return 0;
    for (int cs = 1; cs <= 3; cs++) { const size_t c = (size_t)1 << cs; if (((gx + c - 1) >> cs) * ((gy + c - 1) >> cs) <= CUT_MAX_CELLS) return cs; }
    return 0;
}
#ifndef GSRAST_TAU_BINS
#define GSRAST_TAU_BINS 32
#endif
constexpr int TAU_BINS = GSRAST_TAU_BINS, TAU_COPIES = 4;
struct TauBins { uint32_t lo; float scale ; float inv_scale; uint32_t wave_mask ; };
__host__ __device__ inline uint32_t tau_bin_of(uint32_t key, const TauBins& tb)
{
    if (key <= tb.lo) return 0u;
    const float f = (float)(key - tb.lo) * tb.scale;
    return f >= (float)(TAU_BINS - 1) ? (uint32_t)(TAU_BINS - 1) : (uint32_t)f;
}
__host__ __device__ inline uint32_t tau_bin_far_edge(uint32_t b, const TauBins& tb)
{
    const float e = (float)(b + 1u) * tb.inv_scale;
    const unsigned long long k = (unsigned long long)tb.lo + (unsigned long long)e + 2ull * (b + 2u);
    return k >= (unsigned long long)ZH_KEY_TOP ? ZCUT_NONE : (uint32_t)k;
}
constexpr uint32_t LATE_BIT = 0x80000000u;
constexpr int GATE_WORDS = 80;

constexpr int RS_THREADS = 256;
constexpr uint32_t RS_SELF_SCAN_BLOCKS = 64;
constexpr int RS_ITEMS = 16;
constexpr int RS_CHUNK = RS_THREADS * RS_ITEMS;
constexpr int SC_CHUNK = 4096;

static inline size_t align256(size_t x) { return (x + 255) & ~(size_t)255; }
static inline size_t rs_blocks(size_t n) { return (n + RS_CHUNK - 1) / RS_CHUNK; }
#ifndef GSRAST_DEPTH_ITEMS
#define GSRAST_DEPTH_ITEMS 8
#endif
#ifndef GSRAST_RUN_SORT_ITEMS
#define GSRAST_RUN_SORT_ITEMS 8
#endif
static inline size_t rs_blocks_n(size_t n, int items) { return (n + (size_t)RS_THREADS * items - 1) / ((size_t)RS_THREADS * items); }
static inline size_t scan_tmp_elems(size_t n)
{
    size_t tot = 0;
    while (n > SC_CHUNK) { n = (n + SC_CHUNK - 1) / SC_CHUNK; tot += 2 * (align256(n * 4) / 4); }
    return tot + 512;
}

static inline GeomLayout geom_layout(size_t P)
{
    GeomLayout L; Carver c;
    size_t Pp = P ? P : 1;
    if (REC_STRIDE == 4) { L.rec0 = c.take(Pp * 64); L.rec1 = L.rec0 + 16; L.rec2 = L.rec0 + 32; }
    else { L.rec0 = c.take(Pp * 16); L.rec1 = c.take(Pp * 16); L.rec2 = c.take(Pp * 16); }
    L.cov3D = c.take(Pp * 24); L.clamped = c.take(Pp); L.tiles = c.take(Pp * 4); L.rect = c.take(Pp * 8); L.binrec = c.take(Pp * 32);
    L.keyA = c.take(Pp * 4); L.keyB = c.take(Pp * 4); L.valA = c.take(Pp * 4); L.valB = c.take(Pp * 4);
    L.offsets = c.take(Pp * 4); L.woffsets = c.take(Pp * 4);
    size_t hist_n = 256 * rs_blocks_n(Pp, GSRAST_DEPTH_ITEMS);
    L.hist = c.take(hist_n * 4);
    size_t st = scan_tmp_elems(hist_n) > scan_tmp_elems(Pp) ? scan_tmp_elems(hist_n) : scan_tmp_elems(Pp);
    L.scan_tmp = c.take(st * 4);
    L.scalars = c.take(256);
    L.grec = c.take(Pp * GREC * 4);
    L.keyC = c.take(Pp * 4); L.valC = c.take(Pp * 4);
    L.sort_minmax = c.take(2 * rs_blocks_n(Pp, GSRAST_DEPTH_ITEMS) * 4);
    L.shdA = c.take(Pp * 16); L.shdB = c.take(Pp * 16); L.shdC = c.take(Pp * 4);
    L.zhist = c.take(ZH_COPIES * ZH_BINS * 4);
    {
        const size_t nb = Pp >= BUCKET_SORT_MIN_P ? depth_buckets_host(Pp) : 0;
        L.bk_count = c.take(nb * 8 * 4);
        L.bk_ccount = c.take(8 * 256 * 4);
        L.bk_slab = c.take(nb * GSRAST_BK_CAP * 16);
        L.bk_order = c.take(nb * GSRAST_BK_CAP * 4); L.bk_wincl = c.take(nb * GSRAST_BK_CAP * 4);
        L.bk_info = c.take(nb * 16); L.bk_base = c.take(nb * 4); L.bk_key = c.take((nb + 1) * 4);
        L.bk_order_e = c.take(nb * GSRAST_BK_CAP * 4); L.bk_wincl_e = c.take(nb * GSRAST_BK_CAP * 4); L.bk_info_e = c.take(nb * 16); L.bk_base_e = c.take(nb * 4);
    }
    L.color_skip = c.take(((Pp + 63) / 64) * 8 + 256);
    L.cand_bits = c.take(((Pp + 63) / 64) * 8 + 256);
    L.skip2 = c.take(((Pp + 63) / 64) * 8 + 256);
    L.untouched = c.take(Pp + 256);
    L.total = c.o + 256;
    return L;
}
static inline BinLayout bin_layout(size_t R)
{
    BinLayout L; Carver c;
    size_t Rp = R ? R : 1;
    L.valA = c.take(Rp * 4); L.valB = c.take(Rp * 4); L.keyA = c.take(Rp * 4); L.keyB = c.take(Rp * 4);
    size_t hist_n = 256 * rs_blocks(Rp);
    L.hist = c.take(hist_n * 4);
    L.scan_tmp = c.take(scan_tmp_elems(hist_n) * 4);
    L.total = c.o + 256;
    return L;
}
#ifndef GSRAST_RUNS_PER_BLOCK
#define GSRAST_RUNS_PER_BLOCK 512
#endif
#ifndef GSRAST_RUN_ITEMS
#define GSRAST_RUN_ITEMS 8
#endif
constexpr int RUNS_PER_BLOCK = GSRAST_RUNS_PER_BLOCK;
constexpr int RUN_ITEMS = GSRAST_RUN_ITEMS;
constexpr int RUN_CHUNK = RUN_ITEMS * 256;
struct RunBinLayout {
    size_t point_list, rkeyA, rkeyB, rvalA, rvalB, hist_x, hist_y, scan_tmp, total;
};
static inline RunBinLayout runbin_layout(size_t capR, size_t capQ)
{
    RunBinLayout L; Carver c;
    if (!capR) capR = 1;
    if (!capQ) capQ = 1;
    L.point_list = c.take(2 * capR * 4);
    L.rkeyA = c.take(capQ * 2); L.rkeyB = c.take(capQ * 2); L.rvalA = c.take(capQ * 8); L.rvalB = c.take(capQ * 8);
    L.hist_x = c.take(256 * rs_blocks_n(capQ, GSRAST_RUN_SORT_ITEMS) * 4);
    L.hist_y = c.take(256 * ((capQ + RUNS_PER_BLOCK - 1) / RUNS_PER_BLOCK) * 4);
    L.scan_tmp = c.take((scan_tmp_elems(capQ) + 512) * 4);
    L.total = c.o + 256;
    return L;
}

static inline ImgLayout img_layout(size_t W, size_t H)
{
    ImgLayout L; Carver c;
    size_t N = W * H ? W * H : 1;
    size_t T = ((W + TILE_X - 1) / TILE_X) * ((H + TILE_Y - 1) / TILE_Y);
    if (!T) T = 1;
    L.final_T = c.take(N * 4); L.n_contrib = c.take(N * 4); L.ranges = c.take(T * 8); L.tile_max = c.take(T * 4);
    L.order_fwd = c.take(T * 4); L.order_bwd = c.take(T * 4);
    const size_t Tg = xcd_group_tiles_host((W + TILE_X - 1) / TILE_X, (H + TILE_Y - 1) / TILE_Y);
    L.bucket_cnt = c.take(((XCD_GROUPS + 1) * WORK_BUCKETS + GATE_WORDS) * 4);
    L.bucket_list = c.take(T <= BUCKET_MAX_TILES ? (XCD_GROUPS * WORK_BUCKETS * (Tg ? Tg : 1) + WORK_BUCKETS * T) * 2 : 0);
    L.zcut_used = c.take(T * 4);
    L.tile_flags = c.take(T);
    L.tau_hist = c.take((size_t)TAU_COPIES * T * TAU_BINS * 4);
    L.total = c.o + 256;
    return L;
}
static inline int tile_bits(size_t T)
{
    int bits = 1;
    while (((size_t)1 << bits) < T) bits++;
    return bits;
}
static inline int tile_passes(size_t T)
{
    int p = (tile_bits(T) + 7) / 8;
    return p ? p : 1;
}

#if defined(__HIPCC__)

__device__ __forceinline__ uint32_t work_bucket(uint32_t w)
{
    if (w == 0u) return WORK_BUCKETS - 1;
    const int e = 31 - __builtin_clz(w);
    const uint32_t key = 2u * (uint32_t)e + (e >= 1 ? ((w >> (e - 1)) & 1u) : 0u);
    return key >= (uint32_t)WORK_BUCKETS - 2u ? 0u : (uint32_t)WORK_BUCKETS - 2u - key;
}
__device__ __forceinline__ uint32_t xcd_group_tiles(uint32_t gx, uint32_t ntiles) { return gx * ((ntiles / gx + XCD_GROUPS - 1) / XCD_GROUPS); }
__device__ __forceinline__ unsigned lane_id() { return __builtin_amdgcn_mbcnt_hi(~0u, __builtin_amdgcn_mbcnt_lo(~0u, 0u)); }

template <int MODE, bool BOUNDED = false>
__device__ __forceinline__ float gs_exp(float x)
{
    if constexpr (MODE == 0) {
        if constexpr (!BOUNDED) {
            if (x < -80.0f) return 0.0f;
            x = x > 80.0f ? 80.0f : x;
        }
        float n = __builtin_rintf(x * 1.44269504088896341f);
        float r = __builtin_fmaf(n, -0.693359375f, x);
        r = __builtin_fmaf(n, 2.12194440e-4f, r);
        float p = 1.9875691500e-4f;
        p = __builtin_fmaf(p, r, 1.3981999507e-3f);
        p = __builtin_fmaf(p, r, 8.3334519073e-3f);
        p = __builtin_fmaf(p, r, 4.1665795894e-2f);
        p = __builtin_fmaf(p, r, 1.6666665459e-1f);
        p = __builtin_fmaf(p, r, 5.0000001201e-1f);
        float y = __builtin_fmaf(p, r * r, r) + 1.0f;
        return __builtin_amdgcn_ldexpf(y, (int)n);
    } else if constexpr (MODE == 1) {
        return expf(x);
    } else {
        return __builtin_amdgcn_exp2f(x * 1.44269504088896341f);
    }
}

__device__ __forceinline__ float gs_power(float cx, float cy, float cz, float dx, float dy)
{
    float q = __builtin_fmaf(cz * dy, dy, (cx * dx) * dx);
    return __builtin_fmaf(-0.5f, q, -((cy * dx) * dy));
}

template <int CTRL, int ROW_MASK = 0xf, int BANK_MASK = 0xf>
__device__ __forceinline__ float dpp_add(float v)
{
    int t = __builtin_amdgcn_update_dpp(0, __float_as_int(v), CTRL, ROW_MASK, BANK_MASK, true);
    return v + __int_as_float(t);
}
__device__ __forceinline__ float wave_sum_to_lane63(float v)
{
    v = dpp_add<0x111>(v);
    v = dpp_add<0x112>(v);
    v = dpp_add<0x114>(v);
    v = dpp_add<0x118>(v);
    v = dpp_add<0x142>(v);
    v = dpp_add<0x143>(v);
    return v;
}

template <int CTRL>
__device__ __forceinline__ float dpp_pair_sum(float v)
{
    int t = __builtin_amdgcn_update_dpp(0, __float_as_int(v), CTRL, 0xf, 0xf, false);
    return v + __int_as_float(t);
}
__device__ __forceinline__ float wave_sum8_transposed(const float (&v)[8], unsigned lane)
{
    const bool b0 = lane & 1u, b1 = lane & 2u, b2 = lane & 4u;
    float w[4], x[2];
#pragma unroll
    for (int i = 0; i < 4; i++) {
        const float a = dpp_pair_sum<0xB1>(v[2 * i]);
        const float b = dpp_pair_sum<0xB1>(v[2 * i + 1]);
        w[i] = b0 ? b : a;
    }
#pragma unroll
    for (int i = 0; i < 2; i++) {
        const float a = dpp_pair_sum<0x4E>(w[2 * i]);
        const float b = dpp_pair_sum<0x4E>(w[2 * i + 1]);
        x[i] = b1 ? b : a;
    }
    const float a = dpp_pair_sum<0x124>(x[0]);
// ... 54 lines not shown
```

### saro-gs_amd/csrc/gsrast_host.h

```cpp
#pragma once
#include <hip/hip_runtime.h>
#include <atomic>
#include <cstdio>
#include <type_traits>
#include "../../include/gsrast.h"

namespace gsrast {

struct Carver {
    size_t o = 0;
    size_t take(size_t bytes) { const size_t r = o; o = (o + bytes + 255) & ~(size_t)255; return r; }
};

int fail(int code, const char* what, hipError_t e = hipSuccess);
inline int refuse(const char* who, const char* what)
{
    char msg[160];
    snprintf(msg, sizeof msg, "%s: %s", who, what);
    return fail(GSRAST_E_ARG, msg);
}
#define GS_HIP(call)                                                                  \
    do {                                                                              \
        hipError_t e_ = (call);                                                       \
        if (e_ != hipSuccess) return ::gsrast::fail(GSRAST_E_DEVICE, #call, e_);      \
    } while (0)
int post_launch(const char* what, hipStream_t s);
#define GS_LAUNCHED(what)                                 \
    do {                                                  \
        int rc_ = ::gsrast::post_launch(what, s);         \
        if (rc_ != GSRAST_OK) return rc_;                 \
    } while (0)

struct OptionWords {
    std::atomic<int> exp_mode, binning, tile_clip, cull, lpt, speculative, fwd_pixels_per_lane, bwd_pixels_per_lane, sh_grad_factors, side_stream, depth_sort, forward_only,
                     no_order_hint, dense_backward, no_list_cut, profile, debug_sync, debug_state, ablate, mutate, list_cut_always, chain_gate, touch_bits, sparse_grec,
                     late_fill_min_p, tau_sample, tau_cut, two_level, two_level_min_p, sort_hint, bwd_transposed, hexplane_scatter;
    OptionWords();
};
extern OptionWords g_opt;
gsrast_options snapshot_defaults();

enum KernelId { K_PREPROCESS_FWD, K_SORT_DEPTH, K_SCAN_TILES, K_EMIT, K_SORT_TILE, K_RANGES, K_BLEND_FWD,
                K_BLEND_BWD, K_PREPROCESS_BWD, K_MARK_VISIBLE, K_LOSS_FWD, K_LOSS_BWD, K_COLOR, K_SH_DERIVS, K_CUT_REDO, K_LATE_ZERO, K_GREC_ZERO,
                K_DENSIFY_CLASSIFY, K_DENSIFY_SCAN, K_DENSIFY_APPLY, K_DENSIFY_STATS, K_CONTRIB_BLEND, K_CONTRIB_FINISH, K_FEATURES_FWD, K_FEATURES_BWD, K_DISTORT_FWD, K_DISTORT_BWD, K_ADAM_VISIBLE,
                K_MCMC_PLAN, K_MCMC_SAMPLE, K_MCMC_APPLY, K_MCMC_NOISE, K_MLP_FWD, K_MLP_BWD, K_COUNT };
static_assert(K_MCMC_NOISE == 31, "the ids with a bit of their own");
struct RoctxRange { bool on; explicit RoctxRange(const char* name); ~RoctxRange(); };
struct ProfScope {
    int id; hipStream_t s; hipEvent_t a = nullptr, b = nullptr; bool on; RoctxRange range;
    ProfScope(int id_, hipStream_t s_);
    ~ProfScope();
};

template <typename T> T* at(char* base, size_t off) { return reinterpret_cast<T*>(base + off); }
template <typename T> const T* at(const char* base, size_t off) { return reinterpret_cast<const T*>(base + off); }

template <int V> using int_c = std::integral_constant<int, V>;
template <int V, int... Vs, class F>
void pick_int(int v, F&& f)
{
    if constexpr (sizeof...(Vs) == 0) f(int_c<V>{});
    else if (v == V) f(int_c<V>{});
    else pick_int<Vs...>(v, f);
}
template <class F>
void pick_bool(bool b, F&& f) { if (b) f(std::true_type{}); else f(std::false_type{}); }

int radix_passes(int bits);
int sort_pairs_small(uint32_t* kA, uint32_t* vA, uint32_t* kB, uint32_t* vB, uint32_t n, int bits, uint32_t* hist, uint32_t* scan_tmp, hipStream_t s);
int sort_pairs_large(uint32_t* kA, uint32_t* vA, uint32_t* kB, uint32_t* vB, uint32_t n, int bits, uint32_t* hist, uint32_t* scan_tmp, hipStream_t s);

}
```

### saro-gs_amd/csrc/gsrast_policy.h

```cpp
#pragma once
#include <stdint.h>
#include <algorithm>
#include <atomic>
#include "../../include/gsrast.h"
#include "gsrast_common.h"
#include "gsrast_preprocess.h"

namespace gsrast {

inline void dec_to_zero(std::atomic<int>& a) { int v = a.load(); while (v > 0 && !a.compare_exchange_weak(v, v - 1)) { } }

struct CutPolicy {
    static constexpr uint32_t MIN_RUNS = 1500000u;
    static constexpr int PAUSE = 64;
    static constexpr int SMALL_STREAK = 4;
    static constexpr int MARGIN_MIN = 6, MARGIN_MAX = 16;
    static constexpr int TAU_MIN = 10, TAU_MAX = 96;
    static constexpr int TAU_FORCE = 512;

    std::atomic<int> pause{0};
    std::atomic<uint32_t> pause_P{0};
    std::atomic<int> fb_score{0}, fb_pause{0}, ok_streak{0}, small_streak{0};
    std::atomic<int> margin{MARGIN_MIN}, margin_streak{0}, tau_req{TAU_MIN}, tau_force{0}, tau_streak{0}, tau_min{TAU_MIN};
    std::atomic<int> pass_rate{0};
    std::atomic<uint32_t> passes_reported{0};

    std::atomic<uint32_t> scene_P{0};
    bool begin_forward(uint32_t P)
    {
        const uint32_t pp = pause_P.load();
        if (pause.load() > 0 && (pp > P ? pp - P : P - pp) > pp / 8) pause = 0;
        const uint32_t sp = scene_P.load();
        if (sp == 0u) { scene_P = P; return false; }
        if ((sp > P ? sp - P : P - sp) > sp / 8) {
            scene_P = P;
            fb_score = 0; fb_pause = 0; ok_streak = 0; small_streak = 0; margin = MARGIN_MIN; margin_streak = 0;
            tau_req = tau_min.load(); tau_force = 0; tau_streak = 0; pass_rate = 0;
            return true;
        }
        return false;
    }
    bool pays(uint32_t last_Q, bool always) const { return always || (last_Q >= MIN_RUNS && pause.load() == 0); }
    void sits_out() { dec_to_zero(pause); }
    bool forced_prediction() { const bool f = tau_force.load() > 0; dec_to_zero(tau_force); return f; }
    void forward_counts(bool predicted_available, uint32_t n_late, uint32_t Q, uint32_t Q_early, uint32_t P, bool always)
    {
        if (always) return;
        if ((n_late != 0u || predicted_available) && Q - Q_early < MIN_RUNS) {
            if (++small_streak >= SMALL_STREAK) { small_streak = 0; pause = PAUSE; pause_P = P; }
        } else small_streak = 0;
    }
    static int pass_points(uint32_t q2, uint32_t qall)
    {
        qall = std::max(qall, 8u);
        const uint32_t lo = qall / 8u;
        return q2 <= lo ? 0 : (int)std::min<uint64_t>(8u, ((uint64_t)(q2 - lo) * 8u + lo - 1u) / lo);
    }
    int completion_pass(uint32_t q2, uint32_t qall, uint32_t P, bool always, bool predicted_available)
    {
        const int pts = pass_points(q2, qall);
        passes_reported++;
        if (pts == 0 && fb_score.load() > 0) fb_score--;
        if (pts >= 4) ok_streak = 0;
        { const int m = margin.load(); if (m < MARGIN_MAX) margin = std::min(MARGIN_MAX, m + 2); margin_streak = 0; }
        { const int r = tau_req.load(); if (r < TAU_MAX) tau_req = std::min(TAU_MAX, r + 8); tau_streak = 0; }
        if (predicted_available && (pts >= 2 || (pass_rate += 8) >= 24)) { tau_force = TAU_FORCE; pass_rate = 0; }
        if ((fb_score += pts) >= 16 && !always) {
            const int prev = fb_pause.load(), len = prev <= 0 ? 64 : (prev >= 512 ? 1024 : prev * 2);
            fb_pause = len; pause = len; pause_P = P; fb_score = 8;
        }
        return pts;
    }
    void clean_cut_forward()
    {
        if (fb_score.load() > 0) fb_score--;
        dec_to_zero(pass_rate);
        if (++ok_streak >= 64) fb_pause = 0;
        if (++margin_streak >= 128) { margin_streak = 0; const int m = margin.load(); if (m > MARGIN_MIN) margin = m - 1; }
        if (++tau_streak >= 64) { tau_streak = 0; const int r = tau_req.load(), lo = tau_min.load(); if (r > lo) tau_req = std::max(lo, r - 2); }
    }
};

struct DepthRange {
    std::atomic<uint32_t> klo{ZH_KLO_DEFAULT}; std::atomic<int> shift{ZH_SHIFT_DEFAULT}; std::atomic<uint32_t> khi{0};
    bool coarse() const { return shift.load() == ZH_SHIFT_DEFAULT && klo.load() == ZH_KLO_DEFAULT; }
    bool learn(uint32_t zb, uint32_t call_klo, int call_shift)
    {
        if (zb == 0xFFFFFFFFu) return true;
        const uint32_t first = zb & 0xFFFFu, last = zb >> 16;
        const long long top = ZH_KEY_TOP, bot = ZH_KLO_DEFAULT;
        long long kmin = std::max(zh_bin_start(first, call_klo, call_shift), bot), kmax = std::min(zh_bin_start(last + 1u, call_klo, call_shift), top);
        if (kmax <= kmin) kmax = kmin + 1;
        const long long span = kmax - kmin;
        const bool was_coarse = call_shift == ZH_SHIFT_DEFAULT && call_klo == ZH_KLO_DEFAULT;
        const bool clipped = first == 0u || last >= (uint32_t)ZH_BINS - 1u;
        const long long pad_lo = first == 0u ? 4 * span : span / 8 + 1, pad_hi = last >= (uint32_t)ZH_BINS - 1u ? 4 * span : span / 8 + 1;
        long long lo = std::max(kmin - pad_lo, bot), hi = std::min(kmax + pad_hi, top);
        if (!was_coarse) {
            const uint32_t khi_prev = khi.load();
            const long long plo = call_klo, phi = khi_prev > call_klo ? (long long)khi_prev : (long long)call_klo + ((long long)ZH_MID << call_shift);
            lo = lo < plo ? lo : plo + (lo - plo) / 8;
            hi = hi > phi ? hi : phi - (phi - hi) / 8;
        }
        int sh = 0;
        while (((hi - lo) >> sh) >= (long long)ZH_MID) sh++;
        klo = (uint32_t)lo; shift = sh; khi = (uint32_t)hi;
        return !was_coarse && !clipped;
    }
};

struct DepthSortPolicy {
    std::atomic<int> skip{0};
    std::atomic<int> backoff{0}, clean{0};
    std::atomic<int> depth_short{0};
    void radix_forward() { dec_to_zero(skip); }
    void clean_forward() { if (clean.load() < 1024 && ++clean >= 64) backoff = 0; }
    int overflow(bool table_held)
    {
        const int clean_before = clean.exchange(0);
        if (table_held && (clean_before < 32 || backoff.load() > 0)) {
            const int prev = backoff.load(), next = prev <= 0 ? 16 : (prev >= 2048 ? 4096 : prev * 2);
            backoff = next; skip = next;
        }
        depth_short = 0;
        return skip.load();
    }
    void radix_key_bits(uint32_t bits) { depth_short = bits <= 24u ? 1 : 0; }
};

inline uint32_t grow_capacity(uint32_t v) { const uint64_t w = (uint64_t)v + v / 4 + 4096; return w > 0x7FFFFFFFull ? 0x7FFFFFFFu : (uint32_t)w; }
inline uint32_t follow_hint(uint32_t hint, uint32_t now, int shift) { const uint32_t d = hint - (hint >> shift); return now > d ? now : d; }
inline uint32_t early_launch_runs(uint32_t qe_hint, uint32_t capQ, bool early_set_expected)
{
    if (!qe_hint || !early_set_expected) return capQ;
    return (uint32_t)std::min<uint64_t>(capQ, (uint64_t)qe_hint + qe_hint / 2 + 4096);
}

inline bool options_valid(const gsrast_options& o)
{
    auto ppl_ok = [](int v) { return v == 0 || v == 1 || v == 2 || v == 4; };
    return o.exp_mode >= 0 && o.exp_mode <= 2 && (o.binning == 0 || o.binning == 1) && ppl_ok(o.fwd_pixels_per_lane) && ppl_ok(o.bwd_pixels_per_lane) &&
           o.backward_phase >= 0 && o.backward_phase <= 2 && (o.depth_sort == 0 || o.depth_sort == 1) && (o.dense_backward == 0 || o.dense_backward == 1);
}
inline bool culled_blend(const gsrast_options& o, bool backward) { return o.cull != 0 && (backward || o.fwd_pixels_per_lane == 0); }
struct PlanSwitches { bool list_cut_always, tau_cut, touch_bits, sparse_grec, two_level, chain_gate, sort_hint, debug_state; int two_level_min_p, tau_sample;
                      bool bwd_transposed; int late_fill_min_p, ablate, mutate; };
struct PlanInputs { unsigned flags; int P, W, H, D; bool sh, colors_precomp; int bucket_skip; uint32_t R_hint, last_Q; bool depth_short; };
struct ForwardPlan {
    const char* refusal = nullptr;
    bool aux = false, aa = false;
    bool runbin = false, buckets_ok = false;
    bool bucket_sort = false, two_level = false;
    bool culled = false, ordered = false;
    bool want_hints = false, cut_base = false;
    bool tau_mode = false;
    bool zero_in_blend = false, zero_touched = false;
    bool keep_untouched = false, clip = false, want_shd = false;
    bool spec_eligible = false;
    bool adaptive_sort = false, assume_short = false;
    bool list_cut_always = false, chain_gate = false, debug_state = false; uint32_t tau_sample_mask = 0, T = 0, R_hint = 0, last_Q = 0; int cut_cs = 0;
    bool cut_pays = false, cut = false, tau_forced = false, tau_on = false, pose_known = true, cut_colors = false, speculative = false;
    void policy_answer(bool pays, bool hints_acquired) { cut_pays = pays; cut = cut_base && pays && (hints_acquired || tau_mode); }
    void prediction_answer(bool forced, bool pose_expected) { tau_forced = forced; tau_on = cut && tau_mode && !pose_expected; }
    void pose_answer(bool known) { pose_known = known; cut_colors = cut && zero_in_blend && !debug_state && (known || tau_on); }
    void binning_answer(bool have_buffer) { speculative = spec_eligible && have_buffer; }
};
inline ForwardPlan plan_forward(const gsrast_options& o, const PlanInputs& in, const PlanSwitches& g)
{
    ForwardPlan p;
    p.aux = (in.flags & GSRAST_RENDER_AUX) != 0; p.aa = (in.flags & GSRAST_RENDER_ANTIALIAS) != 0;
    p.culled = culled_blend(o, false);
    if (in.flags & ~(unsigned)(GSRAST_RENDER_AUX | GSRAST_RENDER_ANTIALIAS)) p.refusal = "flags: unknown bits";
    else if (!options_valid(o)) p.refusal = "forward: bad option value";
    else if (p.aux && !p.culled) p.refusal = "forward: acc_depth / alpha need the culled blend kernel (options.cull != 0, fwd_pixels_per_lane == 0)";
    if (p.refusal || in.P <= 0 || in.W <= 0 || in.H <= 0) return p;
    p.list_cut_always = g.list_cut_always; p.tau_mode = g.tau_cut; p.chain_gate = g.chain_gate; p.debug_state = g.debug_state;
    p.tau_sample_mask = (1u << g.tau_sample) - 1u; p.R_hint = in.R_hint; p.last_Q = in.last_Q;
    const size_t P = (size_t)in.P, gx = ((size_t)in.W + TILE_X - 1) / TILE_X, gy = ((size_t)in.H + TILE_Y - 1) / TILE_Y;
    p.T = (uint32_t)gx * (uint32_t)gy;
    p.runbin = o.binning == 0 && gy <= 256 && p.T <= 65536u;
    p.buckets_ok = p.T <= BUCKET_MAX_TILES;
    p.bucket_sort = p.runbin && o.depth_sort == 0 && P >= BUCKET_SORT_MIN_P && in.bucket_skip == 0;
    p.two_level = p.bucket_sort && g.two_level && P >= (size_t)g.two_level_min_p;
    p.ordered = p.culled && o.lpt != 0;
    const bool bucket_order = p.runbin && p.buckets_ok && p.ordered;
    p.want_hints = bucket_order && !o.no_order_hint;
    p.cut_cs = cut_cell_shift(gx, gy);
    p.cut_base = bucket_order && p.bucket_sort && o.tile_clip != 0 && !o.no_list_cut && p.cut_cs != 0 && o.speculative != 0 && in.R_hint != 0;
    p.zero_in_blend = p.culled && P * 4 <= 0xFFFFFFFFull;
    p.keep_untouched = p.culled && !o.forward_only && g.touch_bits;
    p.zero_touched = p.keep_untouched && p.zero_in_blend && g.sparse_grec;
    p.clip = p.runbin && o.tile_clip != 0;
    p.want_shd = in.sh && !in.colors_precomp && in.D > 0 && !o.forward_only;
    p.spec_eligible = p.runbin && o.speculative != 0;
    p.adaptive_sort = rs_blocks_n(P, GSRAST_DEPTH_ITEMS) > RS_SELF_SCAN_BLOCKS;
    p.assume_short = p.adaptive_sort && g.sort_hint && in.depth_short;
    return p;
}

struct BackwardInputs { unsigned flags; int P, D, R, W, H; bool raw_family, sh, colors_precomp, cov3D_precomp, aux_grads ;
                        unsigned known_flags = GSRAST_RENDER_AUX | GSRAST_RENDER_ANTIALIAS;
                        bool abs_sink = false, pose_out = false, pose_scratch = false; };
inline unsigned backward_known_flags(size_t struct_size)
{
    return GSRAST_RENDER_AUX | GSRAST_RENDER_ANTIALIAS | (struct_size >= GSRAST_BACKWARD_CALL_ABS ? GSRAST_RENDER_ABSGRAD : 0u) |
           (struct_size >= sizeof(gsrast_backward_call) ? GSRAST_RENDER_POSEGRAD : 0u);
}
struct BlendBwdPick { int ppl = 1; bool cull = false, transposed = false, aux = false; int ablate = 0; bool abs = false; };
struct BackwardPlan {
    const char* refusal = nullptr;
    bool aux = false, aa = false;
    bool abs = false;
    bool pose = false;
    bool do_blend = false, do_geom = false;
    bool use_sh = false, use_sr = false;
    bool zero_records = false;
    bool derivs = false, derivs_side_wanted = false;
    bool late_fill_wanted = false;
    bool skip_zero_rows = false, join_in_front = false;
    bool blend = false, from_buckets = false, tile_order = false;
    BlendBwdPick pick; uint32_t T = 0; int P = 0;
    bool sh_factor = false; int factors = 0;
    bool sparse = false;
    int mutate = 0;
    bool derivs_on_side = false, late_fill = false, grouped = false, join_late = false; int derivs_grid = 0, per_gaussian_grid = 0;
    bool wants_side() const { return derivs_side_wanted || late_fill_wanted; }
    void side_answer(bool acquired)
    {
        derivs_on_side = derivs_side_wanted && acquired; late_fill = late_fill_wanted && acquired; grouped = late_fill;
        join_late = late_fill && !derivs_on_side && !join_in_front;
        derivs_grid = !derivs ? 0 : derivs_on_side ? std::min((P + 63) / 64, 512) : (P + 63) / 64;
        per_gaussian_grid = !do_geom ? 0 : grouped ? (P + PB_GROUP - 1) / PB_GROUP : (P + PP_THREADS - 1) / PP_THREADS;
    }
};
inline BackwardPlan plan_backward(const gsrast_options& o, const BackwardInputs& in, const PlanSwitches& g)
{
    BackwardPlan p;
    const bool aux_flag = (in.flags & GSRAST_RENDER_AUX) != 0;
    p.aux = aux_flag && in.aux_grads; p.aa = (in.flags & GSRAST_RENDER_ANTIALIAS) != 0;
    p.abs = (in.flags & GSRAST_RENDER_ABSGRAD) != 0;
    p.pose = (in.flags & GSRAST_RENDER_POSEGRAD) != 0;
    p.pick.cull = culled_blend(o, true);
    if (in.flags & ~(in.known_flags | GSRAST_RENDER_ABSGRAD)) p.refusal = "flags: unknown bits";
    else if (!options_valid(o)) p.refusal = "backward: bad option value";
    else if (aux_flag && !p.pick.cull) p.refusal = "backward: acc_depth / alpha gradients need the culled blend kernels (options.cull != 0)";
    else if (p.abs && !(in.known_flags & GSRAST_RENDER_ABSGRAD)) p.refusal = "flags: unknown bits (GSRAST_RENDER_ABSGRAD is known only to a call record whose struct_size covers dL_dmean2D_abs)";
    else if (p.abs && !in.abs_sink) p.refusal = "backward: GSRAST_RENDER_ABSGRAD with a NULL dL_dmean2D_abs";
    else if (!p.abs && in.abs_sink) p.refusal = "backward: dL_dmean2D_abs without GSRAST_RENDER_ABSGRAD";
    else if (p.abs && (!p.pick.cull || g.ablate == 1 || g.ablate == 2))
        p.refusal = "backward: GSRAST_RENDER_ABSGRAD needs the transposed blend backward (options.cull != 0, no ablation kernel)";
    else if (p.pose && !in.pose_out) p.refusal = "backward: GSRAST_RENDER_POSEGRAD with a NULL dL_dcamera";
    else if (p.pose && !in.pose_scratch) p.refusal = "backward: GSRAST_RENDER_POSEGRAD with a NULL pose_scratch";
    else if (!p.pose && (in.pose_out || in.pose_scratch)) p.refusal = "backward: dL_dcamera / pose_scratch without GSRAST_RENDER_POSEGRAD";
    if (p.refusal || in.P <= 0 || in.R < 0 || in.W <= 0 || in.H <= 0) return p;
    p.P = in.P; p.do_blend = o.backward_phase != 2; p.do_geom = o.backward_phase != 1;
    p.use_sh = in.sh && !in.colors_precomp; p.use_sr = !in.cov3D_precomp;
    p.zero_records = p.do_blend && (!o.grads_zeroed || o.forward_only);
    p.derivs = p.do_blend && p.use_sh && in.D > 0 && o.forward_only;
    p.derivs_side_wanted = p.derivs && o.side_stream && in.R > 0;
    p.late_fill_wanted = p.do_blend && p.do_geom && in.R > 0 && !o.dense_backward && o.side_stream && (in.P >= g.late_fill_min_p || g.list_cut_always);
    p.skip_zero_rows = g.ablate == 3; p.join_in_front = g.ablate == 5;
    p.T = (uint32_t)((in.W + TILE_X - 1) / TILE_X) * (uint32_t)((in.H + TILE_Y - 1) / TILE_Y);
    const int forced = o.bwd_pixels_per_lane;
    p.pick.ppl = forced ? forced : p.T >= 32768 ? 4 : (p.T >= 8192 ? 2 : 1);
    p.pick.aux = p.aux; p.pick.abs = p.abs;
    p.pick.ablate = (!p.aux && (g.ablate == 1 || g.ablate == 2)) ? g.ablate : 0;
    p.pick.transposed = p.aux || p.abs || (p.pick.cull && !p.pick.ablate && p.pick.ppl == 1 && g.bwd_transposed);
    p.blend = p.do_blend && in.R > 0;
    const bool ordered = p.blend && p.pick.cull && o.lpt != 0;
    p.from_buckets = ordered && p.T <= BUCKET_MAX_TILES;
    p.tile_order = ordered && !p.from_buckets;
    p.factors = (p.use_sh && o.sh_grad_factors) ? 1 : 0;
    p.sh_factor = p.do_blend && p.factors;
    p.sparse = !o.dense_backward;
    p.mutate = p.blend ? g.mutate : 0;
    return p;
}

}
```

Baseline: 809.3 views/s.

## Defer late-bit Gaussians in two-level bucket refine until the cut redo pass

Adds a REFINE_EARLY mode to the two-level depth-bucket refine. In this mode late elements are not scattered into the fine slab; only their count, weight sum and tile sum go into per-bucket late statistics, which the bucket sort folds into its totals. A REFINE_LATE pass appends the late elements into the slab only when the full sort or the cut redo path actually needs them, and it is predicated on the redo flag. The aim is to cut the scatter and sort work of the early pass, at the price of an extra kernel launch and extra per-bucket state when the late list is needed.

```diff
diff --git a/saro-gs_amd/csrc/gsrast_binning.h b/saro-gs_amd/csrc/gsrast_binning.h
--- a/saro-gs_amd/csrc/gsrast_binning.h
+++ b/saro-gs_amd/csrc/gsrast_binning.h
@@ -648,13 +648,21 @@
     }
 }
 
+constexpr int REFINE_ALL = 0, REFINE_EARLY = 1, REFINE_LATE = 2;
 __global__ void __launch_bounds__(256)
 depth_bucket_refine_kernel(const uint4* __restrict__ cslab , const uint32_t* __restrict__ gccount , uint32_t nb,
-                           uint32_t* __restrict__ gcount , uint4* __restrict__ slab , uint32_t ccap)
+                           uint32_t* gcount , uint4* __restrict__ slab , uint32_t ccap,
+                           int mode = REFINE_ALL, uint4* __restrict__ bk_late = nullptr , const uint32_t* __restrict__ pred = nullptr)
 {
     __shared__ uint32_t cnt[1 << BK_CSHIFT];
+    __shared__ uint32_t late[3][1 << BK_CSHIFT];
+    if (pred && *pred == 0u) return;
     const uint32_t x = blockIdx.x & (BK_XCD - 1), c = blockIdx.x >> 3;
-    if (threadIdx.x < (1u << BK_CSHIFT)) cnt[threadIdx.x] = 0u;
+    uint32_t* const gc = gcount + (size_t)x * nb + (c << BK_CSHIFT);
+    if (threadIdx.x < (1u << BK_CSHIFT)) {
+        cnt[threadIdx.x] = mode == REFINE_LATE ? gc[threadIdx.x] : 0u;
+        late[0][threadIdx.x] = 0u; late[1][threadIdx.x] = 0u; late[2][threadIdx.x] = 0u;
+    }
     const uint32_t n_true = gccount[(size_t)x * BK_NBC_MAX + c];
     const uint32_t n = n_true < ccap ? n_true : ccap;
     const uint4* src = cslab + ((size_t)c * BK_XCD + x) * ccap;
@@ -669,15 +677,23 @@
             const uint32_t e = e0 + r * 256 + threadIdx.x;
             if (e < n) {
                 const uint32_t fb = (el[r].z >> 16) & ((1u << BK_CSHIFT) - 1u);
-                const uint32_t pos = atomicAdd(&cnt[fb], 1u);
-                if (pos < (uint32_t)BK_CAPX)
-                    slab[((size_t)((c << BK_CSHIFT) + fb) * BK_XCD + x) * BK_CAPX + pos] = make_uint4(el[r].x, el[r].y, el[r].z & ~BK_FINE_MASK, el[r].w);
+                const bool is_late = (el[r].z & LATE_BIT) != 0u;
+                if (mode == REFINE_EARLY && is_late) {
+                    atomicAdd(&late[0][fb], 1u); atomicAdd(&late[1][fb], el[r].z & ~(LATE_BIT | BK_FINE_MASK)); atomicAdd(&late[2][fb], el[r].w);
+                } else if (mode != REFINE_LATE || is_late) {
+                    const uint32_t pos = atomicAdd(&cnt[fb], 1u);
+                    if (pos < (uint32_t)BK_CAPX)
+                        slab[((size_t)((c << BK_CSHIFT) + fb) * BK_XCD + x) * BK_CAPX + pos] = make_uint4(el[r].x, el[r].y, el[r].z & ~BK_FINE_MASK, el[r].w);
+                }
             }
         }
     }
     __syncthreads();
-    if (threadIdx.x < (1u << BK_CSHIFT))
-        gcount[(size_t)x * nb + (c << BK_CSHIFT) + threadIdx.x] = (n_true > ccap && threadIdx.x == 0u) ? 0xFFFFu : cnt[threadIdx.x];
+    if (threadIdx.x < (1u << BK_CSHIFT)) {
+        gc[threadIdx.x] = (n_true > ccap && threadIdx.x == 0u && mode != REFINE_LATE) ? 0xFFFFu : cnt[threadIdx.x];
+        if (mode != REFINE_ALL)
+            bk_late[(size_t)x * nb + (c << BK_CSHIFT) + threadIdx.x] = make_uint4(late[0][threadIdx.x], late[1][threadIdx.x], late[2][threadIdx.x], 0u);
+    }
 }
 
 __device__ __forceinline__ void wave_sync() { __builtin_amdgcn_fence(__ATOMIC_ACQ_REL, "wavefront"); __builtin_amdgcn_wave_barrier(); }
@@ -699,6 +715,7 @@
                          uint4* __restrict__ binfo ,
                          uint32_t* __restrict__ bwsum ,
                          uint4* __restrict__ binfo_all = nullptr,
+                         const uint4* __restrict__ bk_late = nullptr,
                          const uint32_t* __restrict__ pred = nullptr ,
                          const unsigned long long* __restrict__ keep_bits = nullptr,
                          uint32_t* __restrict__ zero_words = nullptr, uint32_t n_zero_words = 0,
@@ -727,7 +744,8 @@
         return d < (uint32_t)BK_SUB ? d : (uint32_t)BK_SUB - 1u;
     };
     uint32_t c = lane < (unsigned)BK_XCD ? gcount[(size_t)lane * nb + b] : 0u;
-    const uint32_t over = __ballot(c > (uint32_t)BK_CAPX) != 0ull ? 1u : 0u;
+    const uint4 lt = (bk_late && lane < (unsigned)BK_XCD) ? bk_late[(size_t)lane * nb + b] : make_uint4(0u, 0u, 0u, 0u);
+    const uint32_t over = __ballot(c + lt.x > (uint32_t)BK_CAPX) != 0ull ? 1u : 0u;
     c = c < (uint32_t)BK_CAPX ? c : (uint32_t)BK_CAPX;
     uint32_t inc = c;
 #pragma unroll
@@ -739,7 +757,7 @@
     const uint32_t n_all = start[BK_XCD];
     for (uint32_t k = lane; k <= (uint32_t)BK_SUB; k += 64) cnt[k] = 0u;
     wave_sync();
-    uint32_t tsum = 0, wall = 0;
+    uint32_t tsum = lt.z, wall = lt.y, nlate = lt.x;
     for (uint32_t e0 = lane; e0 < n_all; e0 += 64 * 4) {
         uint4 kv[4];
 #pragma unroll
@@ -798,13 +816,13 @@
     uint32_t run = wave_incl_scan(wsum) - wsum;
     const uint32_t wtot = __shfl(run + wsum, 63, 64);
 #pragma unroll
-    for (int d = 32; d >= 1; d >>= 1) { tsum += __shfl_xor(tsum, d, 64); wall += __shfl_xor(wall, d, 64); }
+    for (int d = 32; d >= 1; d >>= 1) { tsum += __shfl_xor(tsum, d, 64); wall += __shfl_xor(wall, d, 64); nlate += __shfl_xor(nlate, d, 64); }
     uint32_t* scanbuf = reinterpret_cast<uint32_t*>(grp);
     for (uint32_t e = 0; e < E; e++) { const uint32_t t = lane * E + e; if (t < n) { run += aux[t]; scanbuf[t] = run; } }
     wave_sync();
     for (uint32_t t = lane; t < n; t += 64) bwincl[(size_t)b * BK_CAP + t] = scanbuf[t];
     if (lane == 0) {
-        if (early_only) { binfo[b] = make_uint4(n, wtot, n_all - n, over); binfo_all[b] = make_uint4(n_all, wall, tsum, over); }
+        if (early_only) { binfo[b] = make_uint4(n, wtot, n_all - n + nlate, over); binfo_all[b] = make_uint4(n_all + nlate, wall, tsum, over); }
         else binfo[b] = make_uint4(n, wtot, tsum, over);
         bwsum[b] = wtot;
     }
diff --git a/saro-gs_amd/csrc/gsrast_capi.hip b/saro-gs_amd/csrc/gsrast_capi.hip
--- a/saro-gs_amd/csrc/gsrast_capi.hip
+++ b/saro-gs_amd/csrc/gsrast_capi.hip
@@ -65,6 +65,7 @@
     { "tau_cut", &g_opt.tau_cut, 1, OPT_FLAG, 0, 0, nullptr },
     { "two_level", &g_opt.two_level, 1, OPT_FLAG, 0, 0, nullptr },
     { "two_level_min_p", &g_opt.two_level_min_p, 2500000, OPT_CLAMP, 0, OPT_MAX, nullptr },
+    { "refine_early", &g_opt.refine_early, 1, OPT_FLAG, 0, 0, nullptr },
     { "sort_hint", &g_opt.sort_hint, 1, OPT_FLAG, 0, 0, nullptr },
     { "bwd_transposed", &g_opt.bwd_transposed, 1, OPT_FLAG, 0, 0, nullptr },
     { "hexplane_scatter", &g_opt.hexplane_scatter, 0, OPT_ONE_OF, OPT_01, 0, nullptr },
@@ -84,7 +85,7 @@
     const OptionWords& g = g_opt;
     return PlanSwitches{ g.list_cut_always.load() != 0, g.tau_cut.load() != 0, g.touch_bits.load() != 0, g.sparse_grec.load() != 0, g.two_level.load() != 0, g.chain_gate.load() != 0,
                          g.sort_hint.load() != 0, g.debug_state.load() != 0, g.two_level_min_p.load(), g.tau_sample.load(), g.bwd_transposed.load() != 0, g.late_fill_min_p.load(),
-                         g.ablate.load(), g.mutate.load() };
+                         g.ablate.load(), g.mutate.load(), g.refine_early.load() != 0 };
 }
 
 const char* const kKernelNames[K_COUNT] = { "preprocess_fwd", "sort_depth", "scan_tiles", "emit_instances",
@@ -767,6 +768,7 @@
                           p.keep_untouched, p.clip, p.want_shd, p.spec_eligible, p.adaptive_sort, p.assume_short, p.cut_pays, p.cut };
     int v = 0;
     for (size_t k = 0; k < sizeof bits / sizeof bits[0]; k++) v |= bits[k] ? 1 << k : 0;
+    if (words[5] & 2) v |= p.refine_early ? 1 << 19 : 0;
     return v;
 }
 
@@ -885,12 +887,13 @@
 struct BucketSortArgs {
     const uint4* slab; const uint32_t* gcount; uint32_t nb; const uint32_t* bkey; uint32_t *border, *bwincl; uint4* binfo; uint32_t* bwsum;
     uint4* binfo_all = nullptr;
+    const uint4* bk_late = nullptr;
     const uint32_t* pred = nullptr; const unsigned long long* keep_bits = nullptr;
     uint32_t* zero_words = nullptr; uint32_t n_zero_words = 0; uint4* zero_quads = nullptr; uint32_t n_zero_quads = 0;
 };
 void launch_bucket_sort(hipStream_t s, const BucketSortArgs& a)
 {
-    depth_bucket_sort_kernel<<<(a.nb + BK_WAVES - 1) / BK_WAVES, 64 * BK_WAVES, 0, s>>>(a.slab, a.gcount, a.nb, a.bkey, a.border, a.bwincl, a.binfo, a.bwsum, a.binfo_all, a.pred, a.keep_bits,
+    depth_bucket_sort_kernel<<<(a.nb + BK_WAVES - 1) / BK_WAVES, 64 * BK_WAVES, 0, s>>>(a.slab, a.gcount, a.nb, a.bkey, a.border, a.bwincl, a.binfo, a.bwsum, a.binfo_all, a.bk_late, a.pred, a.keep_bits,
                                                                                    a.zero_words, a.n_zero_words, a.zero_quads, a.n_zero_quads);
 }
 struct EmitArgs {
@@ -920,7 +923,7 @@
     int P = 0, W = 0, H = 0; uint32_t T = 0, nbk = 0; CamArgs cam;
     GeomLayout GL; ImgLayout IL; char *geom = nullptr, *img = nullptr, *bin = nullptr; uint32_t cap = 0, capQ = 0;
     float4 *rec0, *rec1, *rec2, *binrec, *grec; uint32_t* tiles; uint2* rect; uint32_t *kA, *kB, *vA, *vB, *offsets, *woffsets, *hist, *scan_tmp, *scalars, *hint_sel, *prefilter_word;
-    uint4 *bk_slab, *bk_info, *bk_info_e; uint32_t *bk_count, *bk_key, *bk_order, *bk_wincl, *bk_base, *bk_order_e, *bk_wincl_e, *bk_base_e;
+    uint4 *bk_slab, *bk_info, *bk_info_e, *bk_late; uint32_t *bk_count, *bk_key, *bk_order, *bk_wincl, *bk_base, *bk_order_e, *bk_wincl_e, *bk_base_e;
     unsigned long long *color_skip, *cand_bits; unsigned char *untouched = nullptr, *tile_flags; uint32_t* bucket_cnt; uint16_t* bucket_list; uint2* ranges;
     uint32_t *zcut_used = nullptr, *tau_hist = nullptr, *zhist_call = nullptr; TauBins tau_bins{};
     HintTable* hints = nullptr;
@@ -933,6 +936,7 @@
     bool bucketed = false;
     bool totals_pending = false;
     bool sort_redone = false;
+    bool late_refined = false;
     Readback *rb_pre = nullptr, *rb_flag = nullptr, *rb = nullptr; uint32_t *pre_alias = nullptr, *flag_alias = nullptr; uint32_t pre_seq = 0, flag_seq = 0;
     ChainGate* gate = nullptr; uint32_t gseq = 0, *gdone = nullptr, *gpred = nullptr;
     uint32_t counts[kCountWords] = { 0 }; uint32_t nQ1 = 0;
@@ -991,7 +995,7 @@
         offsets = at<uint32_t>(geom, GL.offsets); woffsets = at<uint32_t>(geom, GL.woffsets); hist = at<uint32_t>(geom, GL.hist); scan_tmp = at<uint32_t>(geom, GL.scan_tmp);
         scalars = at<uint32_t>(geom, GL.scalars); hint_sel = scalars + HINT_SEL;
         bk_slab = at<uint4>(geom, GL.bk_slab); bk_info = at<uint4>(geom, GL.bk_info); bk_info_e = at<uint4>(geom, GL.bk_info_e);
-        bk_count = at<uint32_t>(geom, GL.bk_count); bk_key = at<uint32_t>(geom, GL.bk_key);
+        bk_count = at<uint32_t>(geom, GL.bk_count); bk_key = at<uint32_t>(geom, GL.bk_key); bk_late = at<uint4>(geom, GL.bk_late);
         bk_order = at<uint32_t>(geom, GL.bk_order); bk_wincl = at<uint32_t>(geom, GL.bk_wincl); bk_base = at<uint32_t>(geom, GL.bk_base);
         bk_order_e = at<uint32_t>(geom, GL.bk_order_e); bk_wincl_e = at<uint32_t>(geom, GL.bk_wincl_e); bk_base_e = at<uint32_t>(geom, GL.bk_base_e);
         color_skip = at<unsigned long long>(geom, GL.color_skip); cand_bits = at<unsigned long long>(geom, GL.cand_bits);
@@ -1071,6 +1075,14 @@
     }
 
     BucketSortArgs whole_buckets() const { return BucketSortArgs{ bk_slab, bk_count, nbk, bk_key, bk_order, bk_wincl, bk_info, bk_base }; }
+    int append_late(hipStream_t s, const uint32_t* pred)
+    {
+        if (!plan.refine_early || !bucketed || late_refined) return GSRAST_OK;
+        late_refined = true;
+        depth_bucket_refine_kernel<<<(nbk >> BK_CSHIFT) * BK_XCD, 256, 0, s>>>(reinterpret_cast<const uint4*>(grec), at<uint32_t>(geom, GL.bk_ccount), nbk, bk_count, bk_slab,
+                                                                             depth_coarse_cap((size_t)P, nbk), REFINE_LATE, bk_late, pred);
+        return post_launch("depth_bucket_refine", s);
+    }
     int sort_and_scan(hipStream_t s, bool assume, bool buckets)
     {
         bucketed = buckets; totals_pending = false;
@@ -1087,11 +1099,11 @@
                                                                            zcut_used, T, (uint32_t)cam.gx, scalars + SC_N_LATE, plan.cut ? color_skip : nullptr, (uint32_t)plan.cut_cs, ccap);
             GS_LAUNCHED("depth_bucket_scatter");
             if (two) {
-                depth_bucket_refine_kernel<<<(nbk >> BK_CSHIFT) * BK_XCD, 256, 0, s>>>(cslab, gccount, nbk, bk_count, bk_slab, ccap);
+                depth_bucket_refine_kernel<<<(nbk >> BK_CSHIFT) * BK_XCD, 256, 0, s>>>(cslab, gccount, nbk, bk_count, bk_slab, ccap, plan.refine_early ? REFINE_EARLY : REFINE_ALL, bk_late, nullptr);
                 GS_LAUNCHED("depth_bucket_refine");
             }
             BucketSortArgs a = whole_buckets();
-            if (plan.cut) { a.border = bk_order_e; a.bwincl = bk_wincl_e; a.binfo = bk_info_e; a.bwsum = bk_base_e; a.binfo_all = bk_info; }
+            if (plan.cut) { a.border = bk_order_e; a.bwincl = bk_wincl_e; a.binfo = bk_info_e; a.bwsum = bk_base_e; a.binfo_all = bk_info; a.bk_late = plan.refine_early ? bk_late : nullptr; }
             a.zero_words = zhist_ctx; a.n_zero_words = ZH_COPIES * ZH_BINS;
             if (tau_ctx) { a.zero_quads = reinterpret_cast<uint4*>(tau_ctx); a.n_zero_quads = (uint32_t)((size_t)TAU_COPIES * T * TAU_BINS / 4); }
             launch_bucket_sort(s, a);
@@ -1213,6 +1225,7 @@
                 e.need2 = tile_flags; e.gx_tiles = cam.gx; e.pass2_counts = scalars + SC_PASS2;
             } else if (bucketed) {
                 if (plan.cut) {
+                    { int rc = append_late(s, nullptr); if (rc != GSRAST_OK) return rc; }
                     launch_bucket_sort(s, whole_buckets());
                     GS_LAUNCHED("depth_bucket_sort");
                 }
@@ -1391,8 +1404,9 @@
         const uint32_t* const pred = gate ? gpred : scalars + SC_REDO_PRED;
         ProfScope ps(K_CUT_REDO, s);
         struct Off { Off() { t_prof_off++; } ~Off() { t_prof_off--; } } off;
-        cut_candidates_kernel<<<std::min((P + 255) / 256, 2048), 256, 0, s>>>((uint32_t)P, tiles, rect, tile_flags, T, (uint32_t)cam.gx, color_skip, cand_bits, at<unsigned long long>(geom, GL.skip2), pred);
-        int rc = post_launch("cut_candidates", s);
+        int rc = append_late(s, pred);
+        if (rc == GSRAST_OK) cut_candidates_kernel<<<std::min((P + 255) / 256, 2048), 256, 0, s>>>((uint32_t)P, tiles, rect, tile_flags, T, (uint32_t)cam.gx, color_skip, cand_bits, at<unsigned long long>(geom, GL.skip2), pred);
+        if (rc == GSRAST_OK) rc = post_launch("cut_candidates", s);
         if (rc == GSRAST_OK && plan.cut_colors) rc = color_kernels(s, true, pred);
         if (rc == GSRAST_OK) rc = run_binning(s, capQ, scalars + SC_PASS2, 2, pred, false);
         if (rc == GSRAST_OK) rc = blend(s, at<uint32_t>(bin, 0), true, 2, pred);
diff --git a/saro-gs_amd/csrc/gsrast_common.h b/saro-gs_amd/csrc/gsrast_common.h
--- a/saro-gs_amd/csrc/gsrast_common.h
+++ b/saro-gs_amd/csrc/gsrast_common.h
@@ -22,7 +22,8 @@
         color_skip ,
         cand_bits ,
         skip2 ,
-        untouched , total;
+        untouched ,
+        bk_late , total;
 };
 constexpr int GREC = 16;
 constexpr size_t BUCKET_SORT_MIN_P = 32768;
@@ -202,6 +203,7 @@
     L.cand_bits = c.take(((Pp + 63) / 64) * 8 + 256);
     L.skip2 = c.take(((Pp + 63) / 64) * 8 + 256);
     L.untouched = c.take(Pp + 256);
+    L.bk_late = c.take((Pp >= BUCKET_SORT_MIN_P ? (size_t)depth_buckets_host(Pp) : 0) * 8 * 16);
     L.total = c.o + 256;
     return L;
 }
diff --git a/saro-gs_amd/csrc/gsrast_host.h b/saro-gs_amd/csrc/gsrast_host.h
--- a/saro-gs_amd/csrc/gsrast_host.h
+++ b/saro-gs_amd/csrc/gsrast_host.h
@@ -34,7 +34,7 @@
 struct OptionWords {
     std::atomic<int> exp_mode, binning, tile_clip, cull, lpt, speculative, fwd_pixels_per_lane, bwd_pixels_per_lane, sh_grad_factors, side_stream, depth_sort, forward_only,
                      no_order_hint, dense_backward, no_list_cut, profile, debug_sync, debug_state, ablate, mutate, list_cut_always, chain_gate, touch_bits, sparse_grec,
-                     late_fill_min_p, tau_sample, tau_cut, two_level, two_level_min_p, sort_hint, bwd_transposed, hexplane_scatter;
+                     late_fill_min_p, tau_sample, tau_cut, two_level, two_level_min_p, sort_hint, bwd_transposed, hexplane_scatter, refine_early;
     OptionWords();
 };
 extern OptionWords g_opt;
diff --git a/saro-gs_amd/csrc/gsrast_policy.h b/saro-gs_amd/csrc/gsrast_policy.h
--- a/saro-gs_amd/csrc/gsrast_policy.h
+++ b/saro-gs_amd/csrc/gsrast_policy.h
@@ -144,13 +144,15 @@
 }
 inline bool culled_blend(const gsrast_options& o, bool backward) { return o.cull != 0 && (backward || o.fwd_pixels_per_lane == 0); }
 struct PlanSwitches { bool list_cut_always, tau_cut, touch_bits, sparse_grec, two_level, chain_gate, sort_hint, debug_state; int two_level_min_p, tau_sample;
-                      bool bwd_transposed; int late_fill_min_p, ablate, mutate; };
+                      bool bwd_transposed; int late_fill_min_p, ablate, mutate;
+                      bool refine_early = true; };
 struct PlanInputs { unsigned flags; int P, W, H, D; bool sh, colors_precomp; int bucket_skip; uint32_t R_hint, last_Q; bool depth_short; };
 struct ForwardPlan {
     const char* refusal = nullptr;
     bool aux = false, aa = false;
     bool runbin = false, buckets_ok = false;
     bool bucket_sort = false, two_level = false;
+    bool refine_early_base = false, refine_early = false;
     bool culled = false, ordered = false;
     bool want_hints = false, cut_base = false;
     bool tau_mode = false;
@@ -160,7 +162,7 @@
     bool adaptive_sort = false, assume_short = false;
     bool list_cut_always = false, chain_gate = false, debug_state = false; uint32_t tau_sample_mask = 0, T = 0, R_hint = 0, last_Q = 0; int cut_cs = 0;
     bool cut_pays = false, cut = false, tau_forced = false, tau_on = false, pose_known = true, cut_colors = false, speculative = false;
-    void policy_answer(bool pays, bool hints_acquired) { cut_pays = pays; cut = cut_base && pays && (hints_acquired || tau_mode); }
+    void policy_answer(bool pays, bool hints_acquired) { cut_pays = pays; cut = cut_base && pays && (hints_acquired || tau_mode); refine_early = refine_early_base && cut; }
     void prediction_answer(bool forced, bool pose_expected) { tau_forced = forced; tau_on = cut && tau_mode && !pose_expected; }
     void pose_answer(bool known) { pose_known = known; cut_colors = cut && zero_in_blend && !debug_state && (known || tau_on); }
     void binning_answer(bool have_buffer) { speculative = spec_eligible && have_buffer; }
@@ -190,6 +192,7 @@
     p.zero_in_blend = p.culled && P * 4 <= 0xFFFFFFFFull;
     p.keep_untouched = p.culled && !o.forward_only && g.touch_bits;
     p.zero_touched = p.keep_untouched && p.zero_in_blend && g.sparse_grec;
+    p.refine_early_base = p.two_level && g.refine_early && p.zero_in_blend && (p.zero_touched || o.forward_only);
     p.clip = p.runbin && o.tile_clip != 0;
     p.want_shd = in.sh && !in.colors_precomp && in.D > 0 && !o.forward_only;
     p.spec_eligible = p.runbin && o.speculative != 0;
```

Result: faster. 822.5 views/s (median of 6 runs) (+1.6%).
